# argriffing/raoteh

Hardware: AMD Instinct MI355X
Metric: site log-likelihoods/sec (batched tree pruning) (higher is better)
Workload: dtype f64; 1 GPU; c3: 61-state MG94 codon, 64-leaf balanced tree, 10000 sites/GPU, dense f64 leaf likelihood vectors; encoding=dense, sites_per_gpu=10000, sites_total=10000, states=61, leaves=64, edges=126, batches_rotated=3, reduce=none

## Files before the change

### include/raoteh_hip.h

```cpp
#ifndef RAOTEH_HIP_H
#define RAOTEH_HIP_H

#include <stdint.h>

#ifdef __cplusplus
extern "C" {
#endif

#define RT_OK                0
#define RT_ERR_INVALID      -1
#define RT_ERR_HIP          -2
#define RT_ERR_UNSUPPORTED  -3
#define RT_ERR_NOMEM        -4
#define RT_ERR_RCCL         -5
#define RT_ERR_SINGULAR     -6
#define RT_ERR_ZERO_PROB    -7

#define RT_MAX_STATES      128
#define RT_MAX_EXPECT_STATES 64
#define RT_MAX_EXPECT_STEP_STATES 128
#define RT_MAX_EXPM_STATES 128

#define RT_SITE_OK           0
#define RT_SITE_ZERO_PROB    1
// ... 53 lines not shown

int rt_mcy_esd_get_node_to_pmap(rt_ctx *ctx, int64_t nnodes, int64_t n,
            int64_t nsites, const int64_t *tree_csr_indices,
            const int64_t *tree_csr_indptr, const double *esd_transitions,
            const int64_t *state_mask, const double *obs_likelihood,
            double *subtree_probability);
int rt_mcy_esd_passes(rt_ctx *ctx, int64_t nnodes, int64_t n, int64_t nsites,
            const int64_t *tree_csr_indices, const int64_t *tree_csr_indptr,
            const double *esd_transitions, int64_t *state_mask,
            const double *obs_likelihood, double *subtree_probability);

int rt_mc0_esd_get_node_to_distn(rt_ctx *ctx, int64_t nnodes, int64_t n,
            int64_t nsites, const int64_t *tree_csr_indices,
            const int64_t *tree_csr_indptr, const double *esd_transitions,
            const double *root_distn, const double *subtree_probability,
            double *node_to_distn_array, int32_t *status);

int rt_mc0_esd_get_joint_endpoint_distn(rt_ctx *ctx, int64_t nnodes, int64_t n,
            int64_t nsites, const int64_t *tree_csr_indices,
            const int64_t *tree_csr_indptr, const double *esd_transitions,
            const double *subtree_probability, const double *node_to_distn_array,
            double *joint_distns);

int rt_mjp_esd_expectation_weights(rt_ctx *ctx, int64_t nnodes, int64_t n,
            int64_t nsites, const int64_t *tree_csr_indices,
            const int64_t *tree_csr_indptr, const double *esd_transitions,
            const double *root_distn, const int64_t *state_mask,
            const double *site_weights, double *edge_weights, int32_t *status);

int rt_mjp_esd_expectation_weights_obs(rt_ctx *ctx, int64_t nnodes, int64_t n,
            int64_t nsites, const int64_t *tree_csr_indices,
            const int64_t *tree_csr_indptr, const double *esd_transitions,
            const double *root_distn, int64_t nobs, const int64_t *obs_nodes, int kind,
            const void *data, const double *site_weights, double *edge_weights,
            int32_t *status);

int rt_mjp_frechet_statistics(rt_ctx *ctx, int64_t n, int64_t nedges, const double *Q,
            int64_t nq, const int64_t *q_index, const double *t, const double *W,
            double *dwell, double *trans);


int rt_model_create(rt_ctx *ctx, int64_t nnodes, int64_t n,
            const int64_t *tree_csr_indices, const int64_t *tree_csr_indptr,
            rt_model **model);
int rt_model_destroy(rt_model *model);

int rt_model_set_rates(rt_model *model, const double *Q, int64_t nq,
            const int64_t *node_q, const double *t);
int rt_model_set_rates_spectral(rt_model *model, const double *A, const double *lam,
            const double *B, const double *D, const double *t);
int rt_model_recompute_transitions(rt_model *model);
int rt_model_set_transitions(rt_model *model, const double *esd_transitions);
int rt_model_get_transitions(rt_model *model, double *esd_transitions);
int rt_model_get_expm_info(rt_model *model, int32_t *info );
int rt_model_set_root_distn(rt_model *model, const double *root_distn);

int rt_model_schedule_depth(const rt_model *model);
int rt_model_get_schedule(const rt_model *model, int32_t *ops, int64_t capacity,
            int64_t *nops);
int rt_build_schedule(int64_t nnodes, const int64_t *tree_csr_indices,
            const int64_t *tree_csr_indptr, int32_t *ops ,
            int32_t *depth);
int rt_set_option(const char *key, int64_t value);
int rt_ctx_set_option(rt_ctx *ctx, const char *key, int64_t value);
int rt_jit_source(int64_t nnodes, const int64_t *tree_csr_indices,
            const int64_t *tree_csr_indptr, int64_t n, int64_t nobs,
            const int64_t *obs_nodes, int64_t prefetch, char *buf, int64_t capacity);

int rt_sites_create(rt_model *model, int64_t nsites, int kind, int64_t nobs,
            const int64_t *obs_nodes, const void *data, rt_sites **sites);
int rt_sites_clone(rt_sites *sites, rt_sites **clone);
int rt_sites_jit_wait(rt_sites *sites);
int rt_jit_wait_all(void);
int rt_sites_destroy(rt_sites *sites);
int64_t rt_sites_device_bytes(const rt_sites *sites);
double rt_sites_jit_compile_seconds(const rt_sites *sites);
int rt_debug_jit_global(rt_sites *sites, const char *name, void *dst, int64_t bytes);
const char *rt_sites_kernel_name(const rt_sites *sites);

int rt_prune(rt_model *model, rt_sites *sites);
int rt_step(rt_model *model, rt_sites *sites, int recompute_transitions);
int rt_carry_combine_deal(int64_t nt, int64_t nblocks16, int64_t G, int root_halves,
            int rescale, int partitioned, int multi, int64_t *tile_of);
int rt_expect_step(rt_model *model, rt_sites *sites, int recompute_transitions,
            double *dwell, double *root_posterior, double *trans, int32_t *status);
#define RT_MAX_POSTERIOR_SETS 8
int rt_sites_posteriors(rt_model *model, rt_sites *sites, int recompute_transitions,
            int64_t n_node_sets, const uint64_t *node_sets,
            int64_t n_edge_sets, const uint64_t *edge_sets,
            int64_t n_marginal_nodes, const int64_t *marginal_nodes,
            double *node_values, double *edge_values, double *marginals, int32_t *status);
#define RT_MAX_BRANCH_COEFS 8
int rt_sites_branch_expectations(rt_model *model, rt_sites *sites, int recompute_transitions,
            int64_t n_coefs, const double *coefs, double *values, double *edge_sums,
            int32_t *status);
#define RT_MAX_PROFILE_POINTS 64
int rt_sites_branch_profiles(rt_model *model, rt_sites *sites, int recompute_transitions,
            int64_t npoints, const double *lengths, double *values, double *sums,
            int32_t *status);
int rt_model_get_branch_lengths(rt_model *model, double *t);
int rt_model_nni_moves(const rt_model *model, int32_t *moves, int64_t capacity, int64_t *nmoves);
int rt_tree_nni_moves(int64_t nnodes, const int64_t *tree_csr_indices, const int64_t *tree_csr_indptr,
            int32_t *moves, int64_t capacity, int64_t *nmoves);
int rt_sites_nni_scores(rt_model *model, rt_sites *sites, int recompute_transitions,
            int64_t npoints, const double *lengths, double *values, double *sums,
            int32_t *status);
#define RT_MAX_PLACE_FRACTIONS 8
#define RT_MAX_PLACE_PENDANT   16
int rt_sites_placements(rt_model *model, rt_sites *sites, int recompute_transitions,
            int64_t nqueries, int query_kind, const void *queries,
            int64_t nfractions, const double *fractions,
            int64_t npendant, const double *pendant,
            double *values, double *sums, int32_t *status);
int rt_model_spr_moves(const rt_model *model, int64_t radius, int32_t *moves, int64_t capacity,
            int64_t *nmoves);
int rt_tree_spr_moves(int64_t nnodes, const int64_t *tree_csr_indices, const int64_t *tree_csr_indptr,
            int64_t radius, int32_t *moves, int64_t capacity, int64_t *nmoves);
int rt_sites_spr_scores(rt_model *model, rt_sites *sites, int recompute_transitions,
            int64_t radius, int64_t nfractions, const double *fractions,
            double *values, double *sums, int32_t *status);
#define RT_MAX_SAMPLE_NODES 8192
int rt_sites_sample_states(rt_model *model, rt_sites *sites, int recompute_transitions,
            uint64_t seed, uint64_t first_draw, int64_t ndraws,
            uint8_t *states ,
            int32_t *status );
int rt_sample_states_draw_block(int64_t nnodes);
int rt_sites_map_states(rt_model *model, rt_sites *sites, int recompute_transitions,
            uint8_t *states      ,
            double  *log_joint   ,
            int32_t *status      );
#define RT_MAX_MAPPING_EVENTS 512
int rt_sites_sample_mappings(rt_model *model, rt_sites *sites, int recompute_transitions,
            uint64_t seed, uint64_t first_draw, int64_t ndraws,
            int64_t n_coefs, const double *coefs ,
            uint8_t *states  ,
            double *values   ,
            int32_t *counts  ,
            double *means    ,
            int32_t *status  );
int rt_sites_set_weights(rt_sites *sites, const double *weights);
int rt_sites_get_logliks(rt_sites *sites, double *loglik, int32_t *status);
int rt_sites_get_totals(rt_sites *sites, double totals[3]);

#define RT_MAX_RATE_SETS 64
int rt_model_set_rate_sets(rt_model *model, int64_t K, const double *Q, int64_t nq,
            const int64_t *node_q, const double *t);
int rt_step_multi(rt_model *model, rt_sites *sites, int recompute_transitions);
int rt_sites_get_multi_logliks(rt_sites *sites, double *loglik, int32_t *status);
int rt_sites_get_multi_totals(rt_sites *sites, double *totals, double *weighted_sums);
int rt_sites_multi_mixture(rt_sites *sites, const double *class_weights, double *loglik,
            int32_t *status, double totals[3]);
const char *rt_sites_multi_kernel_name(const rt_sites *sites);

int rt_partition_plan(const int32_t *site_set, int64_t nsites, int64_t nsets, int64_t granule,
            int64_t capacity, int64_t *order, int64_t *slot_of_site, uint8_t *is_pad,
            int32_t *granule_set, int64_t *run_begin, int64_t *padded);
int rt_sites_create_partitioned(rt_model *model, int64_t nsites, int kind, int64_t nobs,
            const int64_t *obs_nodes, const void *data, const int32_t *site_set, int64_t nsets,
            rt_sites **sites);
int rt_step_partitioned(rt_model *model, rt_sites *sites, int recompute_transitions);
int rt_sites_get_partition_totals(rt_sites *sites, double *totals, double *weighted_sums);
int rt_sites_branch_expectations_partitioned(rt_model *model, rt_sites *sites,
            int recompute_transitions, int64_t n_coefs, int coefs_per_set, const double *coefs,
            double *values, double *edge_sums, double *set_edge_sums, int32_t *status);
int rt_sites_branch_profiles_partitioned(rt_model *model, rt_sites *sites, int recompute_transitions,
            int64_t npoints, const double *factors, double *values, double *sums,
// ... 87 lines not shown
```

### raoteh_amd/_lib.py

```python
from __future__ import annotations

import ctypes
import os
from ctypes import (POINTER, c_char_p, c_double, c_int, c_int32,
                    c_int64, c_ubyte, c_void_p)

__all__ = ['HipLibraryError', 'RaotehHipError', 'lib', 'check', 'LIB_PATH']

LIB_PATH = os.environ.get(
    'RAOTEH_HIP_LIB',
    os.path.join(os.path.dirname(os.path.abspath(__file__)), 'libraoteh_hip.so'))

RT_OK = 0
RT_ERR_INVALID = -1
RT_ERR_HIP = -2
RT_ERR_UNSUPPORTED = -3
RT_ERR_NOMEM = -4
RT_ERR_RCCL = -5
RT_ERR_SINGULAR = -6
RT_ERR_ZERO_PROB = -7

RT_OBS_DENSE, RT_OBS_STATE, RT_OBS_MASK = 0, 1, 2
RT_K_EXPM, RT_K_PRUNE, RT_K_REDUCE, RT_K_COMBINE = 0, 1, 2, 3
RT_SITE_ZERO_PROB = 1
# ... 8 lines not shown
RT_MAX_EXPECT_STATES = 64
RT_MAX_EXPECT_STEP_STATES = 128
RT_MAX_RATE_SETS = 64


class HipLibraryError(ImportError):
    """libraoteh_hip.so is missing / not loadable (run __graft_entry__.build())."""


class RaotehHipError(RuntimeError):

    def __init__(self, code, message):
        RuntimeError.__init__(self, '%s (code %d)' % (message, code))
        self.code = code


_p_i64 = POINTER(c_int64)
_p_f64 = POINTER(c_double)
_p_i32 = POINTER(c_int32)

SIGNATURES = {
    'rt_version': (c_int, []),
    'rt_last_error': (c_char_p, []),
    'rt_device_count': (c_int, [POINTER(c_int)]),
    'rt_ctx_create': (c_int, [c_int, POINTER(c_void_p)]),
    'rt_ctx_destroy': (c_int, [c_void_p]),
    'rt_ctx_sync': (c_int, [c_void_p]),
    'rt_ctx_set_timing': (c_int, [c_void_p, c_int]),
    'rt_ctx_reset_timing': (c_int, [c_void_p]),
    'rt_ctx_kernel_time': (c_int, [c_void_p, c_int, POINTER(c_double),
                                   POINTER(c_int64), POINTER(c_char_p)]),
    'rt_expm': (c_int, [c_void_p, c_int64, c_int64, _p_f64, c_int64, _p_i64,
                        _p_f64, _p_f64, _p_i32]),
    'rt_lb_transition_matrix': (c_int, [c_void_p, c_int64, c_int64, _p_f64, _p_f64, _p_f64]),
    'rt_tmjp_get_inhomogeneous_mjp': (c_int, [c_int64, _p_i64, _p_i64, _p_i64, c_int64, _p_i64,
                                              _p_f64, c_double, c_double, c_int64, _p_i64,
                                              _p_f64]),
    'rt_mcy_get_node_to_pset': (c_int, [c_void_p, c_int64, c_int64, _p_i64, _p_i64, _p_i64,
                                        _p_i64, _p_i64]),
    'rt_get_node_to_set': (c_int, [c_void_p, c_int64, c_int64, _p_i64, _p_i64, _p_i64, _p_i64,
                                   _p_i64, _p_i64]),
    'rt_mcy_esd_get_node_to_pset': (c_int, [c_void_p, c_int64, c_int64, c_int64,
                                            _p_i64, _p_i64, _p_f64, _p_i64]),
    'rt_esd_get_node_to_set': (c_int, [c_void_p, c_int64, c_int64, c_int64,
                                       _p_i64, _p_i64, _p_f64, _p_i64]),
    'rt_mcy_esd_get_node_to_pmap': (c_int, [c_void_p, c_int64, c_int64, c_int64,
                                            _p_i64, _p_i64, _p_f64, _p_i64,
                                            _p_f64, _p_f64]),
    'rt_mcy_esd_passes': (c_int, [c_void_p, c_int64, c_int64, c_int64,
                                  _p_i64, _p_i64, _p_f64, _p_i64,
                                  _p_f64, _p_f64]),
    'rt_mc0_esd_get_node_to_distn': (c_int, [c_void_p, c_int64, c_int64, c_int64,
                                             _p_i64, _p_i64, _p_f64, _p_f64,
                                             _p_f64, _p_f64, _p_i32]),
    'rt_mc0_esd_get_joint_endpoint_distn': (c_int, [c_void_p, c_int64, c_int64,
                                                    c_int64, _p_i64, _p_i64,
                                                    _p_f64, _p_f64, _p_f64,
                                                    _p_f64]),
    'rt_mjp_esd_expectation_weights': (c_int, [c_void_p, c_int64, c_int64, c_int64,
                                               _p_i64, _p_i64, _p_f64, _p_f64, _p_i64,
                                               _p_f64, _p_f64, _p_i32]),
    'rt_mjp_esd_expectation_weights_obs': (c_int, [c_void_p, c_int64, c_int64, c_int64,
                                                   _p_i64, _p_i64, _p_f64, _p_f64, c_int64,
                                                   _p_i64, c_int, c_void_p, _p_f64, _p_f64,
                                                   _p_i32]),
    'rt_mjp_frechet_statistics': (c_int, [c_void_p, c_int64, c_int64, _p_f64, c_int64, _p_i64,
                                          _p_f64, _p_f64, _p_f64, _p_f64]),
    'rt_model_create': (c_int, [c_void_p, c_int64, c_int64, _p_i64, _p_i64,
                                POINTER(c_void_p)]),
    'rt_model_destroy': (c_int, [c_void_p]),
    'rt_model_set_rates': (c_int, [c_void_p, _p_f64, c_int64, _p_i64, _p_f64]),
    'rt_model_set_rates_spectral': (c_int, [c_void_p, _p_f64, _p_f64, _p_f64, _p_f64, _p_f64]),
    'rt_expm_spectral': (c_int, [c_void_p, c_int64, c_int64, _p_f64, _p_f64, _p_f64, _p_f64,
                                 _p_f64, _p_f64]),
    'rt_model_recompute_transitions': (c_int, [c_void_p]),
    'rt_model_set_transitions': (c_int, [c_void_p, _p_f64]),
    'rt_model_get_transitions': (c_int, [c_void_p, _p_f64]),
    'rt_model_get_expm_info': (c_int, [c_void_p, _p_i32]),
    'rt_model_set_root_distn': (c_int, [c_void_p, _p_f64]),
    'rt_model_schedule_depth': (c_int, [c_void_p]),
    'rt_model_get_schedule': (c_int, [c_void_p, _p_i32, c_int64, _p_i64]),
    'rt_build_schedule': (c_int, [c_int64, _p_i64, _p_i64, _p_i32, _p_i32]),
    'rt_carry_combine_deal': (c_int, [c_int64, c_int64, c_int64, c_int, c_int, c_int, c_int, _p_i64]),
    'rt_set_option': (c_int, [c_char_p, c_int64]),
    'rt_ctx_set_option': (c_int, [c_void_p, c_char_p, c_int64]),
    'rt_sites_jit_compile_seconds': (c_double, [c_void_p]),
    'rt_sites_kernel_name': (c_char_p, [c_void_p]),
    'rt_debug_jit_global': (c_int, [c_void_p, c_char_p, c_void_p, c_int64]),
    'rt_jit_source': (c_int, [c_int64, _p_i64, _p_i64, c_int64, c_int64, _p_i64, c_int64,
                              c_char_p, c_int64]),
    'rt_sites_create': (c_int, [c_void_p, c_int64, c_int, c_int64, _p_i64,
                                c_void_p, POINTER(c_void_p)]),
    'rt_sites_clone': (c_int, [c_void_p, POINTER(c_void_p)]),
    'rt_sites_jit_wait': (c_int, [c_void_p]),
    'rt_jit_wait_all': (c_int, []),
    'rt_expect_step': (c_int, [c_void_p, c_void_p, c_int, _p_f64, _p_f64, _p_f64, _p_i32]),
    'rt_sites_posteriors': (c_int, [c_void_p, c_void_p, c_int, c_int64, c_void_p, c_int64,
                                    c_void_p, c_int64, _p_i64, _p_f64, _p_f64, _p_f64, _p_i32]),
    'rt_sites_branch_expectations': (c_int, [c_void_p, c_void_p, c_int, c_int64, _p_f64, _p_f64,
                                             _p_f64, _p_i32]),
    'rt_sites_branch_profiles': (c_int, [c_void_p, c_void_p, c_int, c_int64, _p_f64, _p_f64,
                                         _p_f64, _p_i32]),
    'rt_model_get_branch_lengths': (c_int, [c_void_p, _p_f64]),
    'rt_model_nni_moves': (c_int, [c_void_p, _p_i32, c_int64, _p_i64]),
    'rt_tree_nni_moves': (c_int, [c_int64, _p_i64, _p_i64, _p_i32, c_int64, _p_i64]),
    'rt_sites_nni_scores': (c_int, [c_void_p, c_void_p, c_int, c_int64, _p_f64, _p_f64, _p_f64,
                                    _p_i32]),
    'rt_sites_placements': (c_int, [c_void_p, c_void_p, c_int, c_int64, c_int, c_void_p, c_int64,
                                    _p_f64, c_int64, _p_f64, _p_f64, _p_f64, _p_i32]),
    'rt_model_spr_moves': (c_int, [c_void_p, c_int64, _p_i32, c_int64, _p_i64]),
    'rt_tree_spr_moves': (c_int, [c_int64, _p_i64, _p_i64, c_int64, _p_i32, c_int64, _p_i64]),
    'rt_sites_spr_scores': (c_int, [c_void_p, c_void_p, c_int, c_int64, c_int64, _p_f64, _p_f64,
                                    _p_f64, _p_i32]),
    'rt_sites_sample_states': (c_int, [c_void_p, c_void_p, c_int, ctypes.c_uint64,
                                       ctypes.c_uint64, c_int64, POINTER(c_ubyte), _p_i32]),
    'rt_sample_states_draw_block': (c_int, [c_int64]),
    'rt_sites_map_states': (c_int, [c_void_p, c_void_p, c_int, POINTER(c_ubyte), _p_f64, _p_i32]),
    'rt_sites_sample_mappings': (c_int, [c_void_p, c_void_p, c_int, ctypes.c_uint64,
                                         ctypes.c_uint64, c_int64, c_int64, _p_f64,
                                         POINTER(c_ubyte), _p_f64, _p_i32, _p_f64, _p_i32]),
    'rt_sites_set_weights': (c_int, [c_void_p, _p_f64]),
    'rt_sites_destroy': (c_int, [c_void_p]),
    'rt_sites_device_bytes': (c_int64, [c_void_p]),
    'rt_prune': (c_int, [c_void_p, c_void_p]),
    'rt_step': (c_int, [c_void_p, c_void_p, c_int]),
    'rt_sites_get_logliks': (c_int, [c_void_p, _p_f64, _p_i32]),
    'rt_sites_get_totals': (c_int, [c_void_p, _p_f64]),
    'rt_model_set_rate_sets': (c_int, [c_void_p, c_int64, _p_f64, c_int64, _p_i64, _p_f64]),
    'rt_step_multi': (c_int, [c_void_p, c_void_p, c_int]),
    'rt_sites_get_multi_logliks': (c_int, [c_void_p, _p_f64, _p_i32]),
    'rt_sites_get_multi_totals': (c_int, [c_void_p, _p_f64, _p_f64]),
    'rt_sites_multi_mixture': (c_int, [c_void_p, _p_f64, _p_f64, _p_i32, _p_f64]),
    'rt_sites_multi_kernel_name': (c_char_p, [c_void_p]),
    'rt_partition_plan': (c_int, [_p_i32, c_int64, c_int64, c_int64, c_int64, _p_i64, _p_i64,
                                  POINTER(c_ubyte), _p_i32, _p_i64, _p_i64]),
    'rt_sites_create_partitioned': (c_int, [c_void_p, c_int64, c_int, c_int64, _p_i64, c_void_p,
                                            _p_i32, c_int64, POINTER(c_void_p)]),
    'rt_step_partitioned': (c_int, [c_void_p, c_void_p, c_int]),
    'rt_sites_get_partition_totals': (c_int, [c_void_p, _p_f64, _p_f64]),
    'rt_sites_partition_info': (c_int, [c_void_p, _p_i64, _p_i64, _p_i64]),
    'rt_sites_branch_expectations_partitioned': (c_int, [c_void_p, c_void_p, c_int, c_int64, c_int,
                                                         _p_f64, _p_f64, _p_f64, _p_f64, _p_i32]),
    'rt_sites_branch_profiles_partitioned': (c_int, [c_void_p, c_void_p, c_int, c_int64, _p_f64, _p_f64,
                                                     _p_f64, _p_f64, _p_i32]),
    'rt_sites_nni_scores_partitioned': (c_int, [c_void_p, c_void_p, c_int, c_int64, _p_f64, _p_f64,
                                                _p_f64, _p_f64, _p_i32]),
    'rt_sites_spr_scores_partitioned': (c_int, [c_void_p, c_void_p, c_int, c_int64, c_int64, _p_f64,
                                                _p_f64, _p_f64, _p_f64, _p_i32]),
    'rt_sites_placements_partitioned': (c_int, [c_void_p, c_void_p, c_int, c_int64, c_int, c_void_p,
                                                c_int64, _p_f64, c_int64, _p_f64, _p_f64, _p_f64,
                                                _p_f64, _p_f64, _p_i32]),
    'rt_sites_branch_expectations_mixture': (c_int, [c_void_p, c_void_p, c_int, _p_f64, c_int64, c_int,
                                                     _p_f64, _p_f64, _p_f64, _p_f64, _p_f64, _p_f64,
                                                     _p_f64, _p_i32]),
    'rt_sites_branch_profiles_mixture': (c_int, [c_void_p, c_void_p, c_int, _p_f64, c_int64, _p_f64,
                                                 _p_f64, _p_f64, _p_f64, _p_i32]),
    'rt_sites_nni_scores_mixture': (c_int, [c_void_p, c_void_p, c_int, _p_f64, c_int64, _p_f64,
                                            _p_f64, _p_f64, _p_f64, _p_i32]),
    'rt_sites_spr_scores_mixture': (c_int, [c_void_p, c_void_p, c_int, _p_f64, c_int64, c_int64,
                                            _p_f64, _p_f64, _p_f64, _p_f64, _p_i32]),
    'rt_sites_placements_mixture': (c_int, [c_void_p, c_void_p, c_int, _p_f64, c_int64, c_int,
                                            c_void_p, c_int64, _p_f64, c_int64, _p_f64, _p_f64,
                                            _p_f64, _p_f64, _p_f64, _p_i32]),
    'rt_comm_available': (c_int, []),
    'rt_comm_unique_id': (c_int, [POINTER(c_ubyte)]),
    'rt_comm_init': (c_int, [c_void_p, c_int, c_int, POINTER(c_ubyte)]),
# ... 69 lines not shown
```

### raoteh_amd/csrc/api.hip

```cpp
#include "common.h"
#include "partition_plan.h"

#include <algorithm>
#include <atomic>
#include <functional>
#include <cmath>
#include <cstdlib>


static thread_local char g_err[512] = "";

void rt_set_error(const char *fmt, ...)
{
    va_list ap;
    va_start(ap, fmt);
    vsnprintf(g_err, sizeof(g_err), fmt, ap);
    va_end(ap);
}

extern "C" const char *rt_last_error(void) { return g_err; }
extern "C" int rt_version(void) { return 100; }

extern "C" int rt_device_count(int *count)
{
// ... 271 lines not shown
        for (int64_t e = m->indptr[v]; e < m->indptr[v + 1]; ++e) {
            kids[(size_t)v].push_back((int32_t)m->indices[e]);
            m->parent[(size_t)m->indices[e]] = (int32_t)v;
        }
    std::vector<int> need((size_t)N, 0);
    for (int64_t v = N - 1; v >= 0; --v) {
        auto &k = kids[(size_t)v];
        if (k.empty()) continue;
        std::stable_sort(k.begin(), k.end(),
                         [&](int32_t a, int32_t b) { return need[a] > need[b]; });
        int nd = std::max(1, need[k[0]]);
        for (size_t i = 1; i < k.size(); ++i) nd = std::max(nd, 1 + need[k[i]]);
        need[(size_t)v] = nd;
    }
    m->ops.clear();
    m->ops.reserve((size_t)N);
    std::vector<int32_t> acc_slot((size_t)N, -1);
    std::vector<std::pair<int32_t, size_t>> stack;
    stack.emplace_back(0, 0);
    int sp = 0, maxsp = 0;
    while (!stack.empty()) {
        const int32_t v = stack.back().first;
        const size_t ci = stack.back().second;
        auto &k = kids[(size_t)v];
        if (ci < k.size()) {
            stack.back().second = ci + 1;
            stack.emplace_back(k[ci], 0);
            continue;
        }
        stack.pop_back();
        rt_op op;
        op.node = v;
        op.obs = -1;
        op.pop = k.empty() ? -1 : acc_slot[(size_t)v];
        if (!k.empty()) sp -= 1;
        if (stack.empty()) {
            op.dst = -1;
        } else {
            const int32_t p = stack.back().first;
            if (acc_slot[(size_t)p] < 0) {
                acc_slot[(size_t)p] = sp;
                op.dst = sp | 256;
                sp += 1;
                maxsp = std::max(maxsp, sp);
            } else {
                op.dst = acc_slot[(size_t)p];
            }
        }
        m->ops.push_back(op);
    }
    m->max_depth = maxsp;
}

extern "C" int rt_build_schedule(int64_t nnodes, const int64_t *idx, const int64_t *ptr,
                                 int32_t *ops, int32_t *depth)
{
    RT_REQUIRE(nnodes >= 1 && ptr && (idx || nnodes == 1) && ops, "bad arguments");
    RT_REQUIRE(ptr[0] == 0 && ptr[nnodes] == nnodes - 1,
               "tree_csr_indptr does not describe a tree");
    for (int64_t v = 0; v < nnodes; ++v)
        for (int64_t e = ptr[v]; e < ptr[v + 1]; ++e)
            RT_REQUIRE(idx[e] > v && idx[e] < nnodes, "children not in preorder");
    rt_model m;
    m.nnodes = nnodes;
    if (nnodes > 1) m.indices.assign(idx, idx + (nnodes - 1));
    m.indptr.assign(ptr, ptr + nnodes + 1);
    build_schedule(&m);
    memcpy(ops, m.ops.data(), m.ops.size() * sizeof(rt_op));
    if (depth) *depth = m.max_depth;
    return RT_OK;
}

static int64_t pfrag_doubles(const rt_model *m)
{
    const int64_t nops = (int64_t)m->ops.size();
    if (m->n <= 4) return (nops + 1) * m->n * m->n;
    const int64_t nt = (m->n + 15) / 16, kp = ((m->n + 3) / 4 + 1) / 2;
    return nops * nt * kp * 128;
}

static void rate_sets_release(rt_model *m)
{
    rt_rate_sets &r = m->multi;
    hipFree(r.d_Q); hipFree(r.d_qidx); hipFree(r.d_t); hipFree(r.d_info); hipFree(r.d_step_of_node);
    hipFree(r.d_P); hipFree(r.d_Pfrag); hipFree(r.d_Pquad); hipFree(r.d_Pcol);
    r = rt_rate_sets();
}

extern "C" int rt_model_destroy(rt_model *m)
{
    if (!m) return RT_OK;
    if (m->live_batches > 0) {
        rt_set_error("rt_model_destroy: %d site batch(es) of this model are still alive; "
                     "destroy them first", m->live_batches);
        return RT_ERR_INVALID;
    }
    m->ctx->live_models -= 1;
    hipSetDevice(m->ctx->device);
    rt_expect_state_release(m);
    rt_expect_lane_release(m);
    hipStreamSynchronize(m->ctx->stream);
    hipFree(m->d_indices); hipFree(m->d_indptr); hipFree(m->d_ops); hipFree(m->d_P);
    hipFree(m->d_Pfrag); hipFree(m->d_Pquad); hipFree(m->d_Pcol); hipFree(m->d_root); hipFree(m->d_Q); hipFree(m->d_spec); hipFree(m->d_qidx);
    hipFree(m->d_t); hipFree(m->d_info); hipFree(m->d_step_of_node);
    hipFree(m->d_qidx_step); hipFree(m->d_t_step);
    rate_sets_release(m);
    delete m;
    return RT_OK;
}

extern "C" int rt_model_create(rt_ctx *ctx, int64_t nnodes, int64_t n,
                               const int64_t *idx, const int64_t *ptr, rt_model **out)
{
    RT_REQUIRE(ctx && out, "null pointer");
    *out = nullptr;
    RT_REQUIRE(nnodes >= 1 && n >= 1, "bad sizes");
    RT_REQUIRE(n <= RT_MAX_STATES, "n=%lld > %d", (long long)n, RT_MAX_STATES);
    RT_REQUIRE(nnodes < (1ll << 30), "tree too large");
    RT_REQUIRE(ptr && (idx || nnodes == 1), "null array");
    RT_REQUIRE(ptr[0] == 0 && ptr[nnodes] == nnodes - 1,
               "tree_csr_indptr does not describe a tree");
    std::vector<char> seen((size_t)nnodes, 0);
    for (int64_t v = 0; v < nnodes; ++v) {
        RT_REQUIRE(ptr[v + 1] >= ptr[v], "tree_csr_indptr not monotone");
        for (int64_t e = ptr[v]; e < ptr[v + 1]; ++e) {
            RT_REQUIRE(idx[e] > v && idx[e] < nnodes,
                       "child index %lld of node %lld is not in preorder",
                       (long long)idx[e], (long long)v);
            RT_REQUIRE(!seen[(size_t)idx[e]], "node %lld has two parents",
                       (long long)idx[e]);
            seen[(size_t)idx[e]] = 1;
        }
    }
    RT_HIP(hipSetDevice(ctx->device));
    rt_model *m = new (std::nothrow) rt_model();
    if (!m) return RT_ERR_NOMEM;
    m->ctx = ctx;
    ctx->live_models += 1;
    m->nnodes = nnodes;
    m->n = n;
    if (nnodes > 1) m->indices.assign(idx, idx + (nnodes - 1));
    m->indptr.assign(ptr, ptr + nnodes + 1);
    build_schedule(m);
    const size_t nn = (size_t)n * n;
    hipError_t e = hipMalloc((void **)&m->d_indices, std::max<size_t>(8, (nnodes - 1) * 8));
    if (e == hipSuccess) e = hipMalloc((void **)&m->d_indptr, (nnodes + 1) * 8);
    if (e == hipSuccess) e = hipMalloc((void **)&m->d_ops, m->ops.size() * sizeof(rt_op));
    if (e == hipSuccess) e = hipMalloc((void **)&m->d_P, nnodes * nn * 8);
    if (e == hipSuccess) e = hipMalloc((void **)&m->d_Pfrag, pfrag_doubles(m) * 8);
    if (e == hipSuccess) e = hipMemset(m->d_Pfrag, 0, pfrag_doubles(m) * 8);
    if (e == hipSuccess && n > 4 && n <= 32) {
        const size_t bytes = m->ops.size() * (size_t)rt_quad_stride((int)n) * 8;
        e = hipMalloc((void **)&m->d_Pquad, bytes);
        if (e == hipSuccess) e = hipMemset(m->d_Pquad, 0, bytes);
    }
    if (e == hipSuccess) e = hipMalloc((void **)&m->d_root, n * 8);
    if (e == hipSuccess) e = hipMalloc((void **)&m->d_qidx, nnodes * 4);
    if (e == hipSuccess) e = hipMalloc((void **)&m->d_t, nnodes * 8);
    if (e == hipSuccess) e = hipMalloc((void **)&m->d_info, nnodes * 8);
    if (e == hipSuccess && n <= 4) e = hipMalloc((void **)&m->d_qidx_step, nnodes * 4);
    if (e == hipSuccess && n <= 4) e = hipMalloc((void **)&m->d_t_step, nnodes * 8);
    if (e == hipSuccess && nnodes > 1)
        e = hipMemcpy(m->d_indices, idx, (nnodes - 1) * 8, hipMemcpyHostToDevice);
    if (e == hipSuccess) e = hipMemcpy(m->d_indptr, ptr, (nnodes + 1) * 8, hipMemcpyHostToDevice);
    if (e == hipSuccess)
        e = hipMemcpy(m->d_ops, m->ops.data(), m->ops.size() * sizeof(rt_op),
                      hipMemcpyHostToDevice);
    std::vector<int32_t> step_of((size_t)nnodes, -1);
    for (size_t k = 0; k < m->ops.size(); ++k) step_of[(size_t)m->ops[k].node] = (int32_t)k;
    if (e == hipSuccess) e = hipMalloc((void **)&m->d_step_of_node, nnodes * 4);
    if (e == hipSuccess)
        e = hipMemcpy(m->d_step_of_node, step_of.data(), nnodes * 4, hipMemcpyHostToDevice);
    if (e == hipSuccess) e = hipMemset(m->d_P, 0, nnodes * nn * 8);
    if (e == hipSuccess) e = hipMemset(m->d_info, 0, nnodes * 8);
    std::vector<double> ones((size_t)n, 1.0);
    if (e == hipSuccess) e = hipMemcpy(m->d_root, ones.data(), n * 8, hipMemcpyHostToDevice);
    if (e != hipSuccess) {
        rt_set_error("rt_model_create: %s", hipGetErrorString(e));
        rt_model_destroy(m);
        return e == hipErrorOutOfMemory ? RT_ERR_NOMEM : RT_ERR_HIP;
    }
    *out = m;
    return RT_OK;
}

static int model_upload_edge_parameters(rt_model *m, const std::vector<int32_t> &qi,
                                        const std::vector<double> &tt)
{
    if (qi != m->h_qidx) {
        RT_HIP(hipMemcpy(m->d_qidx, qi.data(), m->nnodes * 4, hipMemcpyHostToDevice));
        m->h_qidx = qi;
        if (m->d_qidx_step) {
            std::vector<int32_t> by_step(m->ops.size());
            for (size_t k = 0; k < m->ops.size(); ++k) by_step[k] = qi[(size_t)m->ops[k].node];
            RT_HIP(hipMemcpy(m->d_qidx_step, by_step.data(), by_step.size() * 4, hipMemcpyHostToDevice));
        }
    }
    if (tt != m->h_t) {
        RT_HIP(hipMemcpy(m->d_t, tt.data(), m->nnodes * 8, hipMemcpyHostToDevice));
        m->h_t = tt;
        if (m->d_t_step) {
            std::vector<double> by_step(m->ops.size());
            for (size_t k = 0; k < m->ops.size(); ++k) by_step[k] = tt[(size_t)m->ops[k].node];
            RT_HIP(hipMemcpy(m->d_t_step, by_step.data(), by_step.size() * 8, hipMemcpyHostToDevice));
        }
    }
    return RT_OK;
}

static int model_run_expm(rt_model *m)
{
    rt_reduce_args red;
    const bool carry = rt_take_pending_reduce(m->ctx, &red);
    if (m->spectral) {
        RT_TRY(rt_flush_combine(m->ctx));
        const size_t nn = (size_t)m->n * m->n;
        RT_TRY(rt_launch_spectral(m->ctx, m->n, m->nnodes, m->d_spec, m->d_spec + 2 * nn,
                                  m->d_spec + nn, m->spectral_has_D ? m->d_spec + 2 * nn + m->n
                                                                    : nullptr,
                                  m->d_qidx, m->d_t, m->d_P, m->d_info, m->d_step_of_node,
                                  m->n <= 4 ? 0 : 1, m->d_Pfrag, carry ? &red : nullptr,
                                  m->d_Pquad));
        m->have_P = true;
        m->rates_current = true;
        m->frag_dirty = false;
        return rt_model_pack_pcol(m);
    }
    rt_combine_args comb;
    rt_sites *carried = nullptr;
    RT_TRY(rt_take_pending_combine(m->ctx, rt_expm_carry_groups(m->ctx, m->n, m->nnodes, carry,
                                                                m->d_Pquad != nullptr),
                                   carry ? &red : nullptr, &comb, &carried));
    const int erc = rt_launch_expm(m->ctx, m->n, m->nnodes, m->d_Q, m->d_qidx, m->d_t, m->d_P,
                                   m->d_info, m->d_step_of_node, m->n <= 4 ? 0 : 1, m->d_Pfrag,
                                   carry ? &red : nullptr, m->d_Pquad, 0, carried ? &comb : nullptr);
    if (carried) RT_TRY(rt_carried_combine_done(m->ctx, carried, erc == RT_OK));
    RT_TRY(erc);
    m->have_P = true;
    m->rates_current = true;
    m->frag_dirty = false;
    return rt_model_pack_pcol(m);
}

extern "C" int rt_model_set_rates(rt_model *m, const double *Q, int64_t nq,
                                  const int64_t *node_q, const double *t)
{
    RT_REQUIRE(m && Q && t, "null pointer");
    RT_REQUIRE(nq >= 1, "nq must be >= 1");
    if (m->n > RT_MAX_EXPM_STATES) {
        rt_set_error("expm: n=%lld > %d", (long long)m->n, RT_MAX_EXPM_STATES);
        return RT_ERR_UNSUPPORTED;
    }
    RT_HIP(hipSetDevice(m->ctx->device));
    const size_t nn = (size_t)m->n * m->n;
    std::vector<int32_t> qi((size_t)m->nnodes);
    std::vector<double> tt((size_t)m->nnodes);
    qi[0] = -1;
    tt[0] = 0.0;
    for (int64_t v = 1; v < m->nnodes; ++v) {
        const int64_t q = node_q ? node_q[v] : 0;
        RT_REQUIRE(q >= 0 && q < nq, "node_q[%lld]=%lld out of range", (long long)v,
                   (long long)q);
        RT_REQUIRE(std::isfinite(t[v]), "branch length of node %lld is not finite",
                   (long long)v);
        qi[(size_t)v] = (int32_t)q;
        tt[(size_t)v] = t[v];
    }
    if (nq > m->q_capacity) {
        hipFree(m->d_Q);
        m->d_Q = nullptr;
        m->q_capacity = 0;
        RT_HIP(hipMalloc((void **)&m->d_Q, nq * nn * 8));
        m->q_capacity = nq;
    }
    hipStream_t st = m->ctx->stream;
    RT_HIP(hipStreamSynchronize(st));
    RT_HIP(hipMemcpy(m->d_Q, Q, nq * nn * 8, hipMemcpyHostToDevice));
    RT_TRY(model_upload_edge_parameters(m, qi, tt));
    m->spectral = false;
    return model_run_expm(m);
}

extern "C" int rt_model_set_rates_spectral(rt_model *m, const double *A, const double *lam,
                                           const double *B, const double *D, const double *t)
{
    RT_REQUIRE(m && A && lam && B && t, "null pointer");
    if (m->n > 64) {
        rt_set_error("spectral reconstruction: n=%lld > 64", (long long)m->n);
        return RT_ERR_UNSUPPORTED;
    }
    RT_HIP(hipSetDevice(m->ctx->device));
    const size_t n = (size_t)m->n, nn = n * n;
    std::vector<int32_t> qi((size_t)m->nnodes, 0);
    std::vector<double> tt((size_t)m->nnodes);
    qi[0] = -1;
    tt[0] = 0.0;
    for (int64_t v = 1; v < m->nnodes; ++v) {
        RT_REQUIRE(std::isfinite(t[v]), "branch length of node %lld is not finite", (long long)v);
        tt[(size_t)v] = t[v];
    }
    for (size_t i = 0; i < n; ++i)
        RT_REQUIRE(std::isfinite(lam[i]) && (!D || D[i] >= 0.0), "eigenvalue / weight %zu", i);
    if (!m->d_spec) RT_HIP(hipMalloc((void **)&m->d_spec, (2 * nn + 2 * n) * 8));
    RT_HIP(hipStreamSynchronize(m->ctx->stream));
    RT_HIP(hipMemcpy(m->d_spec, A, nn * 8, hipMemcpyHostToDevice));
    RT_HIP(hipMemcpy(m->d_spec + nn, B, nn * 8, hipMemcpyHostToDevice));
    RT_HIP(hipMemcpy(m->d_spec + 2 * nn, lam, n * 8, hipMemcpyHostToDevice));
    if (D) RT_HIP(hipMemcpy(m->d_spec + 2 * nn + n, D, n * 8, hipMemcpyHostToDevice));
    m->spectral_has_D = D != nullptr;
    RT_TRY(model_upload_edge_parameters(m, qi, tt));
    m->spectral = true;
    return model_run_expm(m);
}

extern "C" int rt_expm_spectral(rt_ctx *ctx, int64_t n, int64_t count, const double *A,
                                const double *lam, const double *B, const double *D,
                                const double *t, double *P)
{
    RT_REQUIRE(ctx, "null context");
    RT_REQUIRE(n >= 1 && count >= 0, "bad sizes");
    RT_REQUIRE(A && lam && B && t && P, "null array");
    if (n > 64) {
        rt_set_error("spectral reconstruction: n=%lld > 64", (long long)n);
        return RT_ERR_UNSUPPORTED;
    }
    if (count == 0) return RT_OK;
    RT_HIP(hipSetDevice(ctx->device));
    const size_t nn = (size_t)n * n;
    auto up = [](size_t b) { return (b + 255) & ~(size_t)255; };
    const size_t o_A = 0, o_B = o_A + up(nn * 8), o_lam = o_B + up(nn * 8), o_D = o_lam + up(n * 8),
                 o_t = o_D + up(n * 8), o_P = o_t + up(count * 8), total = o_P + up(count * nn * 8);
    RT_TRY(rt_scratch_reserve(ctx, total));
    unsigned char *base = ctx->d_scratch;
    double *dA = (double *)(base + o_A), *dB = (double *)(base + o_B), *dl = (double *)(base + o_lam),
           *dD = (double *)(base + o_D), *dt = (double *)(base + o_t), *dP = (double *)(base + o_P);
    int rc = RT_OK;
    hipError_t e = hipMemcpyAsync(dA, A, nn * 8, hipMemcpyHostToDevice, ctx->stream);
    if (e == hipSuccess) e = hipMemcpyAsync(dB, B, nn * 8, hipMemcpyHostToDevice, ctx->stream);
    if (e == hipSuccess) e = hipMemcpyAsync(dl, lam, n * 8, hipMemcpyHostToDevice, ctx->stream);
    if (e == hipSuccess && D) e = hipMemcpyAsync(dD, D, n * 8, hipMemcpyHostToDevice, ctx->stream);
    if (e == hipSuccess) e = hipMemcpyAsync(dt, t, count * 8, hipMemcpyHostToDevice, ctx->stream);
    if (e == hipSuccess)
        rc = rt_launch_spectral(ctx, n, count, dA, dl, dB, D ? dD : nullptr, nullptr, dt, dP, nullptr,
                                nullptr, 0, nullptr);
    if (e == hipSuccess && rc == RT_OK)
        e = hipMemcpyAsync(P, dP, count * nn * 8, hipMemcpyDeviceToHost, ctx->stream);
    if (e == hipSuccess && rc == RT_OK) e = hipStreamSynchronize(ctx->stream);
    if (rc != RT_OK) return rc;
    if (e != hipSuccess) {
        rt_set_error("rt_expm_spectral: %s", hipGetErrorString(e));
        return RT_ERR_HIP;
    }
    return RT_OK;
}


static int64_t rate_sets_steps(const rt_model *m)
{
    return (int64_t)m->ops.size() + (m->n <= 4 ? 1 : 0);
}

static int rate_sets_reserve(rt_model *m, int64_t K, int64_t nq)
{
    rt_rate_sets &r = m->multi;
    const int64_t n = m->n, N = m->nnodes, nn = n * n, nops = (int64_t)m->ops.size();
    if (K * nq > r.q_capacity) {
        RT_HIP(hipStreamSynchronize(m->ctx->stream));
        hipFree(r.d_Q);
        r.d_Q = nullptr;
        r.q_capacity = 0;
        RT_HIP(hipMalloc((void **)&r.d_Q, (size_t)(K * nq * nn) * 8));
        r.q_capacity = K * nq;
    }
    if (K <= r.capacity) return RT_OK;
    RT_HIP(hipStreamSynchronize(m->ctx->stream));
    double *keep_Q = r.d_Q;
    const int64_t keep_cap = r.q_capacity;
    r.d_Q = nullptr;
    const uint64_t epoch = r.epoch;
    rate_sets_release(m);
    r.d_Q = keep_Q;
    r.q_capacity = keep_cap;
    r.epoch = epoch + 1;
    r.P_stride = N * nn;
    r.frag_stride = pfrag_doubles(m);
    r.quad_stride = m->d_Pquad ? nops * (int64_t)rt_quad_stride((int)n) : 0;
    r.pcol_stride = nops * n * 16 * ((n + 15) / 16);
    hipError_t e = hipMalloc((void **)&r.d_qidx, (size_t)(K * N) * 4);
    if (e == hipSuccess) e = hipMalloc((void **)&r.d_t, (size_t)(K * N) * 8);
    if (e == hipSuccess) e = hipMalloc((void **)&r.d_info, (size_t)(K * N) * 8);
    if (e == hipSuccess) e = hipMalloc((void **)&r.d_step_of_node, (size_t)(K * N) * 4);
    if (e == hipSuccess) e = hipMalloc((void **)&r.d_P, (size_t)(K * r.P_stride) * 8);
    if (e == hipSuccess) e = hipMalloc((void **)&r.d_Pfrag, (size_t)(K * r.frag_stride) * 8);
    if (e == hipSuccess) e = hipMemset(r.d_Pfrag, 0, (size_t)(K * r.frag_stride) * 8);
    if (e == hipSuccess && r.quad_stride) {
        e = hipMalloc((void **)&r.d_Pquad, (size_t)(K * r.quad_stride) * 8);
        if (e == hipSuccess) e = hipMemset(r.d_Pquad, 0, (size_t)(K * r.quad_stride) * 8);
    }
    if (e == hipSuccess) e = hipMemset(r.d_info, 0, (size_t)(K * N) * 8);
    std::vector<int32_t> son((size_t)(K * N));
    const int64_t steps = rate_sets_steps(m);
    for (int64_t k = 0; k < K; ++k)
        for (size_t j = 0; j < m->ops.size(); ++j)
            son[(size_t)(k * N + m->ops[j].node)] = (int32_t)(k * steps + (int64_t)j);
    if (e == hipSuccess)
        e = hipMemcpy(r.d_step_of_node, son.data(), son.size() * 4, hipMemcpyHostToDevice);
    if (e == hipSuccess) e = hipDeviceSynchronize();
    if (e != hipSuccess) {
        rt_set_error("rt_model_set_rate_sets: %s", hipGetErrorString(e));
        rate_sets_release(m);
        m->multi.epoch = epoch + 1;
        return e == hipErrorOutOfMemory ? RT_ERR_NOMEM : RT_ERR_HIP;
    }
    r.capacity = K;
    return RT_OK;
}

static int rate_sets_pack_pcol(rt_model *m, bool fresh)
{
    rt_rate_sets &r = m->multi;
    if (!m->d_Pcol || m->n <= 4 || r.K <= 0) return RT_OK;
    if (r.pcol_capacity < r.capacity) {
        RT_HIP(hipStreamSynchronize(m->ctx->stream));
        hipFree(r.d_Pcol);
        r.d_Pcol = nullptr;
        r.pcol_capacity = 0;
        RT_HIP(hipMalloc((void **)&r.d_Pcol, (size_t)(r.capacity * r.pcol_stride) * 8));
        r.pcol_capacity = r.capacity;
        fresh = true;
    }
    if (!fresh) return RT_OK;
    return rt_pack_pcol_sets(m, r.K, r.d_P, r.P_stride, r.d_Pcol, r.pcol_stride);
}

static int rate_sets_run_expm(rt_model *m)
{
    rt_rate_sets &r = m->multi;
    RT_TRY(rt_launch_expm(m->ctx, m->n, r.K * m->nnodes, r.d_Q, r.d_qidx, r.d_t, r.d_P, r.d_info,
                          r.d_step_of_node, m->n <= 4 ? 0 : 1, r.d_Pfrag, nullptr, r.d_Pquad,
                          m->nnodes));
    return rate_sets_pack_pcol(m, true);
}

int rt_rate_sets_recompute(rt_model *m)
{
    RT_REQUIRE(m->multi.K > 0, "rt_model_set_rate_sets has not been called");
    return rate_sets_run_expm(m);
}

extern "C" int rt_model_set_rate_sets(rt_model *m, int64_t K, const double *Q, int64_t nq,
                                      const int64_t *node_q, const double *t)
{
    RT_REQUIRE(m && Q && t, "null pointer");
    RT_REQUIRE(K >= 1 && K <= RT_MAX_RATE_SETS, "K=%lld rate sets: 1..%d", (long long)K,
               RT_MAX_RATE_SETS);
    RT_REQUIRE(nq >= 1, "nq must be >= 1");
    if (m->n > RT_MAX_EXPM_STATES) {
        rt_set_error("expm: n=%lld > %d", (long long)m->n, RT_MAX_EXPM_STATES);
        return RT_ERR_UNSUPPORTED;
    }
    RT_HIP(hipSetDevice(m->ctx->device));
    const int64_t N = m->nnodes;
    const size_t nn = (size_t)m->n * m->n;
    std::vector<int32_t> qi((size_t)(K * N));
    std::vector<double> tt((size_t)(K * N));
    for (int64_t k = 0; k < K; ++k) {
        qi[(size_t)(k * N)] = -1;
        tt[(size_t)(k * N)] = 0.0;
        for (int64_t v = 1; v < N; ++v) {
            const int64_t q = node_q ? node_q[v] : 0;
            RT_REQUIRE(q >= 0 && q < nq, "node_q[%lld]=%lld out of range", (long long)v, (long long)q);
            RT_REQUIRE(std::isfinite(t[k * N + v]),
                       "branch length of node %lld in rate set %lld is not finite", (long long)v,
                       (long long)k);
            qi[(size_t)(k * N + v)] = (int32_t)(k * nq + q);
            tt[(size_t)(k * N + v)] = t[k * N + v];
        }
    }
    RT_TRY(rate_sets_reserve(m, K, nq));
    rt_rate_sets &r = m->multi;
    RT_HIP(hipStreamSynchronize(m->ctx->stream));
    RT_HIP(hipMemcpy(r.d_Q, Q, (size_t)(K * nq) * nn * 8, hipMemcpyHostToDevice));
    RT_HIP(hipMemcpy(r.d_qidx, qi.data(), qi.size() * 4, hipMemcpyHostToDevice));
    RT_HIP(hipMemcpy(r.d_t, tt.data(), tt.size() * 8, hipMemcpyHostToDevice));
    if (K != r.K) r.epoch += 1;
    r.K = K;
    r.nq = nq;
    r.h_node_q.assign((size_t)N, -1);
    for (int64_t v = 1; v < N; ++v) r.h_node_q[(size_t)v] = node_q ? (int32_t)node_q[v] : 0;
    return rate_sets_run_expm(m);
}

extern "C" int rt_model_recompute_transitions(rt_model *m)
{
    RT_REQUIRE(m, "null model");
    RT_REQUIRE(m->d_Q || m->spectral, "rt_model_set_rates has not been called");
    RT_HIP(hipSetDevice(m->ctx->device));
    return model_run_expm(m);
}

extern "C" int rt_model_set_transitions(rt_model *m, const double *esd)
{
    RT_REQUIRE(m && esd, "null pointer");
    RT_HIP(hipSetDevice(m->ctx->device));
    RT_HIP(hipStreamSynchronize(m->ctx->stream));
    RT_HIP(hipMemcpy(m->d_P, esd, (size_t)m->nnodes * m->n * m->n * 8,
                     hipMemcpyHostToDevice));
    m->have_P = true;
    m->rates_current = false;
    m->frag_dirty = true;
    return rt_launch_pfrag(m);
}

extern "C" int rt_model_get_transitions(rt_model *m, double *esd)
{
    RT_REQUIRE(m && esd, "null pointer");
    RT_REQUIRE(m->have_P, "the model has no transition matrices yet");
    RT_HIP(hipSetDevice(m->ctx->device));
    RT_HIP(hipStreamSynchronize(m->ctx->stream));
    RT_HIP(hipMemcpy(esd, m->d_P, (size_t)m->nnodes * m->n * m->n * 8,
                     hipMemcpyDeviceToHost));
    return RT_OK;
}

extern "C" int rt_model_get_expm_info(rt_model *m, int32_t *info)
{
    RT_REQUIRE(m && info, "null pointer");
    RT_HIP(hipSetDevice(m->ctx->device));
    RT_HIP(hipStreamSynchronize(m->ctx->stream));
    RT_HIP(hipMemcpy(info, m->d_info, (size_t)m->nnodes * 8, hipMemcpyDeviceToHost));
    for (int64_t v = 1; v < m->nnodes; ++v)
        if (info[2 * v] < 0) {
            rt_set_error("expm: the matrix of the edge above node %lld has a non-finite entry or "
                         "norm (Taylor scheme), or its Pade denominator is singular "
                         "(RAOTEH_EXPM=pade)", (long long)v);
            return RT_ERR_SINGULAR;
        }
    return RT_OK;
}

extern "C" int rt_model_set_root_distn(rt_model *m, const double *root_distn)
{
    RT_REQUIRE(m, "null model");
    RT_HIP(hipSetDevice(m->ctx->device));
    std::vector<double> w((size_t)m->n, 1.0);
    if (root_distn) w.assign(root_distn, root_distn + m->n);
    RT_TRY(rt_flush_pending(m->ctx));
    RT_HIP(hipStreamSynchronize(m->ctx->stream));
    RT_HIP(hipMemcpy(m->d_root, w.data(), m->n * 8, hipMemcpyHostToDevice));
    return RT_OK;
}

extern "C" int rt_model_schedule_depth(const rt_model *m)
{
    return m ? m->max_depth : -1;
}


static std::atomic<int> g_force_generic{0};
static std::atomic<int> g_jit{-1};
static const int64_t RT_JIT_MIN_WORK = 65536;
static std::atomic<int> g_jit_block_sites{0};
static std::atomic<int> g_jit_async{1};
static std::atomic<int> g_rescale{0};
static std::atomic<int> g_leaf_state_kernels{1};
// ... 1936 lines not shown
```

### raoteh_amd/csrc/common.h

```cpp
#pragma once

#include <hip/hip_runtime.h>
#include <hip/hip_ext.h>

#include <cstdarg>
#include <cstdint>
#include <cstdio>
#include <cstring>
#include <memory>
#include <string>
#include <type_traits>
#include <vector>

#include "../../include/raoteh_hip.h"


void rt_set_error(const char *fmt, ...);

#define RT_HIP(call)                                                          \
    do {                                                                      \
        hipError_t e_ = (call);                                               \
        if (e_ != hipSuccess) {                                               \
            rt_set_error("%s failed: %s (%s:%d)", #call,                      \
                         hipGetErrorString(e_), __FILE__, __LINE__);          \
// ... 30 lines not shown
    {
        for (void *&q : ptrs) if (q == p) q = nullptr;
        return p;
    }
};

struct post_plan {
    size_t total = 0;
    size_t take(size_t bytes)
    {
        const size_t o = total;
        total += (bytes + 255) / 256 * 256;
        return o;
    }
};
template <int LO, int HI, class F>
inline int post_dispatch(int v, F &&f)
{
    if constexpr (LO > HI) return RT_ERR_UNSUPPORTED;
    else return v == LO ? f(std::integral_constant<int, LO>()) : post_dispatch<LO + 1, HI>(v, f);
}

struct rt_jit_job;


struct rt_timing_slot {
    std::vector<std::pair<hipEvent_t, hipEvent_t>> pending;
    std::vector<hipEvent_t> pool;
    double total_ms = 0.0;
    int64_t launches = 0;
    int64_t seen = 0;
    char name[64] = "";
};

static const int RT_TOTALS_SLOTS = 4096;

struct rt_ctx {
    int device = 0;
    hipStream_t stream = nullptr;
    int num_cus = 0;
    bool timing = false;
    int timing_period = 1;
    rt_timing_slot slots[RT_K_COUNT];
    hipEvent_t ev_start = nullptr, ev_stop = nullptr;
    double *d_totals_arena = nullptr;
    std::vector<int> totals_free;
    hipEvent_t ev_reduced = nullptr;
    hipEvent_t comm_events[8] = {};
    int comm_event_next = 0;
    unsigned char *d_scratch = nullptr;
    size_t scratch_bytes = 0;
    void *comm = nullptr;
    hipStream_t comm_stream = nullptr;
    void *rccl = nullptr;
    int opt_force_generic = -2;
    int opt_jit = -2;
    int opt_jit_block_sites = -2;
    int opt_jit_async = -2;
    int opt_rescale = -2;
    int opt_leaf_state_kernels = -2;
    struct rt_sites *pending_reduce = nullptr;
    struct rt_sites *pending_combine = nullptr;
    size_t expm_attr_lds = 0;
    size_t expm_ts_attr_lds[8] = {0, 0, 0, 0, 0, 0, 0, 0};
    size_t expm_split_attr_lds = 0;
    size_t expm_w8_attr_lds[3] = {0, 0, 0};
    size_t expm_wide_attr_lds[8] = {0, 0, 0, 0, 0, 0, 0, 0};
    double *d_expm_scratch = nullptr;
    void *expect_cache = nullptr;
    size_t expm_scratch_bytes = 0;
    int live_models = 0, live_chains = 0;
};
static const int RT_OPT_UNSET = -2;

static const int RT_FAST_MAX_DEPTH = 16;

struct rt_op {
    int32_t node;
    int32_t obs;
    int32_t pop;
    int32_t dst;
};

struct rt_rate_sets {
    int64_t K = 0;
    int64_t capacity = 0;
    int64_t nq = 0, q_capacity = 0;
    uint64_t epoch = 0;
    double *d_Q = nullptr;
    int32_t *d_qidx = nullptr;
    double *d_t = nullptr;
    std::vector<int32_t> h_node_q;
    int32_t *d_info = nullptr;
    int32_t *d_step_of_node = nullptr;
    double *d_P = nullptr;
    double *d_Pfrag = nullptr, *d_Pquad = nullptr, *d_Pcol = nullptr;
    int64_t pcol_capacity = 0;
    int64_t P_stride = 0, frag_stride = 0, quad_stride = 0, pcol_stride = 0;
};

struct rt_model {
    rt_ctx *ctx = nullptr;
    int64_t nnodes = 0;
    int64_t n = 0;
    std::vector<int64_t> indices, indptr;
    std::vector<int32_t> parent;
    std::vector<rt_op> ops;
    std::vector<int32_t> h_qidx;
    std::vector<double> h_t;
    int max_depth = 0;
    int64_t *d_indices = nullptr, *d_indptr = nullptr;
    rt_op *d_ops = nullptr;
    double *d_P = nullptr;
    double *d_Pfrag = nullptr;
    double *d_Pquad = nullptr;
    double *d_Pcol = nullptr;
    double *d_root = nullptr;
    double *d_spec = nullptr;
    bool spectral = false, spectral_has_D = false;
    double *d_Q = nullptr;
    int64_t q_capacity = 0;
    int32_t *d_qidx = nullptr;
    double *d_t = nullptr;
    int32_t *d_info = nullptr;
    int32_t *d_step_of_node = nullptr;
    int32_t *d_qidx_step = nullptr;
    double *d_t_step = nullptr;
    bool have_P = false;
    bool rates_current = false;
    bool frag_dirty = true;
    int live_batches = 0;
    void *expect_state = nullptr;
    void *expect_lane_state = nullptr;
    rt_rate_sets multi;
};

enum { RT_LAYOUT_LANE = 0, RT_LAYOUT_MFMA = 1 };

struct rt_partition {
    int64_t nsites = 0;
    int64_t nsets = 0, G = 0, padded = 0;
    int64_t *d_order = nullptr;
    int64_t *d_slot_of_site = nullptr;
    uint8_t *d_is_pad = nullptr;
    int32_t *d_granule_set = nullptr;
    int64_t *d_run_begin = nullptr;
    std::vector<int64_t> run_begin;
    double *d_loglik = nullptr;
    int32_t *d_status = nullptr;
    int nblocks = 1;
    double *d_totals = nullptr;
    bool stepped = false;
    uint64_t epoch = 0;
    int64_t model_K = 0;
    int64_t device_bytes = 0;
};

struct rt_sites {
    rt_model *model = nullptr;
    int64_t nsites = 0;
    int64_t nobs = 0;
    int layout = RT_LAYOUT_LANE;
    bool lane_dma = false;
    int lane_ring = 8;
    bool mfma_solo = false;
    int64_t nblocks = 0;
    int64_t obs_bytes = 0;
    std::vector<int32_t> node_obs;
    std::vector<rt_op> ops;
    rt_op *d_ops = nullptr;
    int32_t *d_lane_ops = nullptr;
    int lane_stack_slots = 1;
    int64_t lane_nprog = 0;
    double *d_obs = nullptr;
    double *d_loglik = nullptr;
    int32_t *d_status = nullptr;
    double *d_partial = nullptr;
    int64_t npartials = 0;
    double *d_totals = nullptr;
    int totals_slot = -1;
    hipEvent_t ev_comm_done = nullptr;
    bool comm_pending = false;
    void *jit_fn = nullptr;
    int jit_prefetch = 0;
    int jit_lookahead = 1;
    int block_sites = 64;
    int jit_waves = 1;
    int jit_tiles = 1;
    bool jit_quad = false;
    bool jit_fused = false;
    double *d_partial_alt = nullptr;
    bool jit_halves = false;
    void *jit_combine = nullptr;
    double *d_half = nullptr;
    bool jit_fold = false;
    bool jit_teams = false;
    int *d_half_count = nullptr;
    bool interp_halves = false;
    bool rescale = false;
    int32_t *d_lane_ops_a = nullptr, *d_lane_ops_b = nullptr;
    int32_t *d_down_meta = nullptr;
    int down_slots = 0;
    int half_nops[2] = {0, 0};
    int half_rec1 = 0, half_kobs1 = 0, half_kroot = -1;
// ... 9 lines not shown
    int jit_kind = 0;
    bool keep_raw = false;
    void *d_raw = nullptr;
    int *d_raw_src = nullptr;
    struct { int S = 64, WG = 1, D = 1, LA = 1, compact = 0; bool fuse = false; } jit_lane;
    bool sparse_ok = false;
    bool sparse_pairs = false;
    bool jit_sparse = false;
    bool jit_pipe = false;
    unsigned *d_leafw = nullptr;
    double *d_weights = nullptr;
    unsigned char *d_sets = nullptr;
    rt_sites *expect_twin = nullptr;
    bool obs_borrowed = false;
    bool counted = false;
    bool pruned = false;
    char kernel_name[64] = "";
    int64_t multi_capacity = 0;
    int64_t multi_padded = 0, multi_npartials = 0;
    int64_t multi_K = 0;
    uint64_t multi_epoch = 0;
    void *multi_last_fn = nullptr;
    bool multi_last_valid = false;
    double *d_mloglik = nullptr;
    int32_t *d_mstatus = nullptr;
    double *d_mpartial = nullptr;
    double *d_mtotals = nullptr;
    char multi_kernel_name[80] = "";
    int multi_state = 0;
    void *multi_fn = nullptr, *multi_combine = nullptr, *multi_for = nullptr;
    std::shared_ptr<rt_jit_job> multi_job;
    std::string multi_src;
    double *d_mhalf = nullptr;
    int *d_mhalf_count = nullptr;
    int64_t multi_half_stride = 0, multi_count_stride = 0, multi_half_capacity = 0;
    double jit_compile_s = 0.0;
    rt_partition *part = nullptr;
};


void rt_time_begin(rt_ctx *ctx, int kernel, const char *name, hipEvent_t *start);
void rt_time_end(rt_ctx *ctx, int kernel, hipEvent_t start);
bool rt_time_extra_begin(rt_ctx *ctx, int kernel, const char *name, hipEvent_t *a, hipEvent_t *b);
void rt_time_extra_end(rt_ctx *ctx, int kernel, hipEvent_t a, hipEvent_t b);

struct rt_reduce_args {
    const double *partial = nullptr;
    long npartials = 0;
    double *totals = nullptr;
    double nsites = 0.0;
};
struct rt_combine_args {
    const double *halfbuf = nullptr;
    const double *obs = nullptr;
    int K = 0, KP = 0, kroot = -1;
    const double *root_w = nullptr;
    int n = 0;
    double *loglik = nullptr;
    int *status = nullptr;
    double *partial = nullptr;
    long nsites = 0, nblocks16 = 0;
    int wave_slots = 1;
};
__host__ __device__ inline long rt_carry_tile(long wg, int k, long G, long nblocks16)
{
    const long t = wg + (long)k * G;
    return t < nblocks16 ? t : -1;
}
inline bool rt_carry_combine_plan(int64_t nt, int64_t nblocks16, int64_t G, bool halves, bool rescale,
                                  bool partitioned, bool multi, int64_t *tile_of = nullptr)
{
    const bool ok = nt == 4 && halves && !rescale && !partitioned && !multi && G >= 1 &&
                    nblocks16 >= 1 && nblocks16 <= 4 * G;
    if (ok && tile_of)
        for (int64_t wg = 0; wg < G; ++wg)
            for (int k = 0; k < 4; ++k) tile_of[4 * wg + k] = rt_carry_tile((long)wg, k, (long)G, (long)nblocks16);
    return ok;
}
int64_t rt_expm_carry_groups(rt_ctx *ctx, int64_t n, int64_t count, bool with_reduce, bool quad);
int rt_expm_wide_launch(rt_ctx *ctx, int nt, bool split2, size_t grid, int64_t n, const double *d_Q,
                        const int *d_qidx, const double *d_t, double *d_P, int *d_info,
                        const int *d_step_of_node, int frag_kind, double *d_Pfrag,
                        const rt_reduce_args &red);
int rt_launch_expm(rt_ctx *ctx, int64_t n, int64_t count, const double *d_Q,
                   const int32_t *d_qidx, const double *d_t, double *d_P,
                   int32_t *d_info, const int32_t *d_step_of_node, int frag_kind,
                   double *d_Pfrag, const rt_reduce_args *fused_reduce = nullptr,
                   double *d_Pquad = nullptr, int64_t variant_count = 0,
                   const rt_combine_args *carried_combine = nullptr);
int rt_launch_spectral(rt_ctx *ctx, int64_t n, int64_t count, const double *d_A,
                       const double *d_lam, const double *d_B, const double *d_D,
                       const int32_t *d_qidx, const double *d_t, double *d_P, int32_t *d_info,
                       const int32_t *d_step_of_node, int frag_kind, double *d_Pfrag,
                       const rt_reduce_args *fused_reduce = nullptr, double *d_Pquad = nullptr);
bool rt_take_pending_reduce(rt_ctx *ctx, rt_reduce_args *out);
int rt_flush_reduce(rt_ctx *ctx);
int rt_take_pending_combine(rt_ctx *ctx, int64_t G, const rt_reduce_args *red, rt_combine_args *out,
                            struct rt_sites **taken);
int rt_carried_combine_done(rt_ctx *ctx, struct rt_sites *s, bool launched);
int rt_flush_combine(rt_ctx *ctx);
int rt_flush_pending(rt_ctx *ctx);
int rt_flush_pending_of(rt_ctx *ctx, const struct rt_sites *s);
#define RT_LAUNCH_TIMED(ctx, kern, grid, block, lds, ...)                               \
    do {                                                                                \
        if ((ctx)->ev_start)                                                            \
            hipExtLaunchKernelGGL(kern, grid, block, lds, (ctx)->stream,                \
                                  (ctx)->ev_start, (ctx)->ev_stop, 0, __VA_ARGS__);     \
        else                                                                            \
            hipLaunchKernelGGL(kern, grid, block, lds, (ctx)->stream, __VA_ARGS__);     \
    } while (0)
int rt_launch_pfrag(rt_model *m);
int rt_model_pack_pcol(rt_model *m);
int rt_model_need_pcol(rt_model *m);
int rt_pack_pcol_sets(rt_model *m, int64_t sets, const double *d_P, int64_t P_stride, double *d_Pcol,
                      int64_t pcol_stride);
struct rt_prune_view {
    const double *P = nullptr, *Pfrag = nullptr, *Pquad = nullptr, *Pcol = nullptr;
    double *loglik = nullptr;
    int32_t *status = nullptr;
    double *partial = nullptr;
    const int32_t *granule_set = nullptr;
    int64_t frag_stride = 0, pcol_stride = 0;
    bool defer_combine = false;
};
int64_t rt_lane_reg_granule(const rt_model *m);
int rt_partition_stage1_blocks(int64_t longest_run);
int64_t rt_partition_totals_doubles(int64_t nsets, int nblocks);
int rt_partition_reduce_launch(rt_ctx *ctx, const rt_partition *part, const double *d_loglik,
                               const int32_t *d_status, const double *d_weights,
                               double *d_batch_totals);
int64_t rt_multi_totals_doubles(int64_t K, int64_t nsites);
int rt_multi_reduce_launch(rt_ctx *ctx, int64_t K, const double *d_partial, int64_t npartials,
                           const double *d_loglik, const int32_t *d_status, int64_t padded,
                           int64_t nsites, const double *d_weights, double *d_totals,
                           double *d_wsums);
int rt_multi_mixture_launch(rt_ctx *ctx, int64_t K, const double *d_logc, const double *d_loglik,
                            const int32_t *d_status, int64_t padded, int64_t nsites,
                            const double *d_weights, double *d_out, int32_t *d_out_status,
                            double *d_partial, double *d_totals);
int rt_launch_prune(rt_model *m, rt_sites *s, bool defer_reduce = false, bool fuse_expm = false,
                    const struct rt_prune_view *view = nullptr);
struct rt_fuse_args {
    rt_reduce_args red;
    bool expm = false;
};
std::string rt_jit_lane_source(const std::vector<rt_op> &ops, int n, int K, int D, int LA,
                               int S, int WG, int compact = 0, bool fuse = false);
std::string rt_jit_mfma_source(const std::vector<rt_op> &ops, int n, int K, int T, int D, int LA,
                               bool quad = false, int sparse = 0);
std::string rt_jit_mfma_split_source(const std::vector<rt_op> &ops, int n, int K, int T, int D,
                                     int LA, int sparse = 0);
bool rt_jit_fold_enabled();
std::string rt_jit_mfma_split_pipelined_source(const std::vector<rt_op> &ops, int n, int K, int T,
                                               int D, int LA, bool halves = false,
                                               int sparse = 0, bool multi = false,
                                               bool teams = false);
bool rt_jit_teams_possible(int n, int T, int sparse);
int rt_jit_teams_env();
void rt_jit_root_halves(const std::vector<rt_op> &ops, int *stepsA, int *stepsB);
bool rt_split_at_root(const std::vector<rt_op> &ops, std::vector<rt_op> *A, std::vector<rt_op> *B);
int rt_jit_companion(const rt_ctx *ctx, void *fn, const char *name, void **out);
int rt_jit_get(rt_ctx *ctx, const std::string &src, void **fn, bool mfma = false,
               double *compile_s = nullptr);
std::shared_ptr<rt_jit_job> rt_jit_start(rt_ctx *ctx, std::vector<std::string> sources, bool mfma);
bool rt_jit_job_done(rt_jit_job *job, bool wait);
void rt_jit_job_result(rt_jit_job *job, int *rc, int *chosen, double *seconds, std::string *error);
void rt_jit_join_all(const rt_ctx *ctx);
int rt_jit_jobs_pending();
int rt_jit_cached(const rt_ctx *ctx, const std::string &src);
int rt_sites_jit_poll(rt_sites *s, bool wait);
void rt_jit_ref(const rt_ctx *ctx, void *fn, int delta);
int rt_jit_verified(const rt_ctx *ctx, void *fn);
// ... 66 lines not shown
```

### raoteh_amd/csrc/expm.hip

```cpp
#include "common.h"

#include <algorithm>
#include "reduce.h"
#include "site_epilogue.h"
#include "combine_body.inc"

#include <cstdlib>

namespace {

__constant__ double c_theta[5] = {1.495585217958292e-2, 2.539398330063230e-1,
                                  9.504178996162932e-1, 2.097847961257068e0,
                                  5.371920351148152e0};
__constant__ double c_b3[4] = {120., 60., 12., 1.};
__constant__ double c_b5[6] = {30240., 15120., 3360., 420., 30., 1.};
__constant__ double c_b7[8] = {17297280., 8648640., 1995840., 277200.,
                               25200., 1512., 56., 1.};
__constant__ double c_b9[10] = {17643225600., 8821612800., 2075673600.,
                                302702400., 30270240., 2162160., 110880.,
                                3960., 90., 1.};
__constant__ double c_b13[14] = {64764752532480000., 32382376266240000.,
                                 7771770303897600., 1187353796428800.,
                                 129060195264000., 10559470521600.,
                                 670442572800., 33522128640., 1323241920.,
// ... 304 lines not shown
            switch ((k + 1) >> 4) {
            case 0:
#pragma unroll
                for (int a = 0; a < 4; ++a) nb[16 * a] = g[a][0];
                break;
            case 1:
#pragma unroll
                for (int a = 0; a < 4; ++a) nb[16 * a] = g[a][1];
                break;
            case 2:
#pragma unroll
                for (int a = 0; a < 4; ++a) nb[16 * a] = g[a][2];
                break;
            default:
#pragma unroll
                for (int a = 0; a < 4; ++a) nb[16 * a] = g[a][3];
                break;
            }
        }
        __syncthreads();
    }
    __syncthreads();
    if (ibuf[2]) {
        for (int e = tid; e < nn; e += TPB) Pb[e] = __builtin_nan("");
        if (info && tid == 0) info[2 * b] = -1;
        return;
    }
#pragma unroll
    for (int a = 0; a < 4; ++a) {
        const int i = ri + 16 * a;
        if (i < n) {
            const double d = dinv[i];
            const int xr = kof[i];
#pragma unroll
            for (int bb = 0; bb < 8; ++bb) {
                const int c = ci + 16 * bb;
                if (c >= n && c < 2 * n) Xb[xr * ld + (c - n)] = g[a][bb] * d;
            }
        }
    }
    __syncthreads();
    for (int q = 0; q < s; ++q) lds_matmul(Xb, Xb, Xb, n, ld, NT, KS);

    RT_FOR_EACH_ELEMENT(i, j, o_unused_) {
        const int e = i * n + j;
        Pb[e] = Xb[i * ld + j];
    }
    if (step >= 0 && frag_kind == 0) {
        RT_FOR_EACH_ELEMENT(i, j, o_unused_) {
            const int e = i * n + j;
            Pfrag[(long)step * nn + e] = Xb[i * ld + j];
        }
    } else if (step >= 0 && frag_kind == 1) {
        const int KP = (KS + 1) / 2;
        const int total = NT * KP * 128;
        for (int e = tid; e < total; e += TPB) {
            const int e2 = e & 1;
            const int ln = (e >> 1) & 63;
            const int q = (e >> 7) % KP;
            const int mm = (e >> 7) / KP;
            const int row = 16 * mm + (ln & 15);
            const int col = 4 * (2 * q + e2) + (ln >> 4);
            Pfrag[(long)step * total + e] = (row < n && col < n) ? Xb[row * ld + col] : 0.0;
        }
        if (Pquad) {
            const int tq = KS * KS * 16;
            for (int e = tid; e < tq; e += TPB) {
                const int i = e & 3, k = (e >> 2) & 3, blk = e >> 4;
                const int row = 4 * (blk / KS) + i, col = 4 * (blk % KS) + k;
                Pquad[(long)step * rt_quad_stride(n) + e] = (row < n && col < n) ? Xb[row * ld + col] : 0.0;
            }
        }
    }
}


__constant__ double c_theta_taylor[5] = {1.3863479e-5, 9.0656564e-3, 8.9577602e-2,
                                         2.9961589e-1, 6.4108352e-1};
__constant__ double c_inv_fact[16] = {
    1.0, 1.0, 0.5, 1.0 / 6.0, 1.0 / 24.0, 1.0 / 120.0, 1.0 / 720.0, 1.0 / 5040.0,
    1.0 / 40320.0, 1.0 / 362880.0, 1.0 / 3628800.0, 1.0 / 39916800.0, 1.0 / 479001600.0,
    1.0 / 6227020800.0, 1.0 / 87178291200.0, 1.0 / 1307674368000.0};

template <int NT>
struct lane_tiles {
    double v[(NT + 1) / 2][(NT + 1) / 2][4];
};

template <int NT>
__device__ __forceinline__ void load_tiles(const double *M, lane_tiles<NT> &t)
{
    constexpr int RH = (NT + 1) / 2;
    constexpr int LD = 16 * NT + 1;
    const int lane = threadIdx.x & 63;
    const int wave = __builtin_amdgcn_readfirstlane(threadIdx.x >> 6);
    const int wr = wave >> 1, wc = wave & 1;
    const int lr = lane & 15, lq = lane >> 4;
#pragma unroll
    for (int u = 0; u < RH; ++u)
#pragma unroll
        for (int v = 0; v < RH; ++v) {
            const int m = wr * RH + u, j = wc * RH + v;
            const bool ok = m < NT && j < NT;
#pragma unroll
            for (int r = 0; r < 4; ++r)
                t.v[u][v][r] = ok ? M[(16 * m + 4 * r + lq) * LD + 16 * j + lr] : 0.0;
        }
}

template <int NT>
__device__ __forceinline__ void mm_blocked(const double *X, const double *Y, double *C,
                                           const double *cf, const double *P1, const double *P2,
                                           const lane_tiles<NT> *R1 = nullptr,
                                           const lane_tiles<NT> *R2 = nullptr,
                                           lane_tiles<NT> *out = nullptr,
                                           const double *top = nullptr, double *C2 = nullptr)
{
    constexpr int RH = (NT + 1) / 2;
    constexpr int LD = 16 * NT + 1;
    constexpr int KS = 4 * NT;
    const int lane = threadIdx.x & 63;
    const int wave = __builtin_amdgcn_readfirstlane(threadIdx.x >> 6);
    const int wr = wave >> 1, wc = wave & 1;
    const int lr = lane & 15, lq = lane >> 4;
    double4_t acc[RH][RH];
    const double *ap[RH];
    const double *bp[RH];
    bool rok[RH], cok[RH];
#pragma unroll
    for (int u = 0; u < RH; ++u) {
        const int m = wr * RH + u, j = wc * RH + u;
        rok[u] = m < NT;
        cok[u] = j < NT;
        ap[u] = X + (16 * (rok[u] ? m : 0) + lr) * LD + lq;
        bp[u] = Y + lq * LD + 16 * (cok[u] ? j : 0) + lr;
#pragma unroll
        for (int v = 0; v < RH; ++v) acc[u][v] = (double4_t){0.0, 0.0, 0.0, 0.0};
    }
    if (cf) {
        const double c0 = cf[0], c1 = cf[1], c2 = cf[2];
#pragma unroll
        for (int u = 0; u < RH; ++u)
#pragma unroll
            for (int v = 0; v < RH; ++v)
                if (rok[u] && cok[v]) {
                    const int m = wr * RH + u, j = wc * RH + v;
                    const int col = 16 * j + lr;
#pragma unroll
                    for (int r = 0; r < 4; ++r) {
                        const int row = 16 * m + 4 * r + lq;
                        const int o = row * LD + col;
                        double w = c1 * (R1 ? R1->v[u][v][r] : P1[o]);
                        if (R2) w = fma(c2, R2->v[u][v][r], w);
                        else if (P2) w = fma(c2, P2[o], w);
                        if (row == col && (double)row < cf[3]) w += c0;
                        acc[u][v][r] = w;
                    }
                }
    }
    double a0[RH], b0[RH], a1[RH], b1[RH];
#pragma unroll
    for (int u = 0; u < RH; ++u) {
        a0[u] = ap[u][0];
        b0[u] = bp[u][0];
        a1[u] = ap[u][KS > 1 ? 4 : 0];
        b1[u] = bp[u][KS > 1 ? 4 * LD : 0];
    }
    for (int kk = 0; kk < KS; ++kk) {
        const int kn = kk + 2 < KS ? kk + 2 : KS - 1;
        double a2[RH], b2[RH];
#pragma unroll
        for (int u = 0; u < RH; ++u) { a2[u] = ap[u][4 * kn]; b2[u] = bp[u][4 * kn * LD]; }
        __builtin_amdgcn_sched_barrier(0);
#pragma unroll
        for (int u = 0; u < RH; ++u)
#pragma unroll
            for (int v = 0; v < RH; ++v)
                acc[u][v] = __builtin_amdgcn_mfma_f64_16x16x4f64(a0[u], b0[v], acc[u][v], 0, 0, 0);
        __builtin_amdgcn_sched_barrier(0);
#pragma unroll
        for (int u = 0; u < RH; ++u) { a0[u] = a1[u]; b0[u] = b1[u]; a1[u] = a2[u]; b1[u] = b2[u]; }
    }
    if (out) {
#pragma unroll
        for (int u = 0; u < RH; ++u)
#pragma unroll
            for (int v = 0; v < RH; ++v)
#pragma unroll
                for (int r = 0; r < 4; ++r) out->v[u][v][r] = acc[u][v][r];
    }
    __syncthreads();
#pragma unroll
    for (int u = 0; u < RH; ++u)
#pragma unroll
        for (int v = 0; v < RH; ++v)
            if (rok[u] && cok[v]) {
                const int m = wr * RH + u, j = wc * RH + v;
                const int col = 16 * j + lr;
#pragma unroll
                for (int r = 0; r < 4; ++r) {
                    const int row = 16 * m + 4 * r + lq;
                    C[row * LD + col] = acc[u][v][r];
                    if (top) {
                        double w = top[1] * R1->v[u][v][r];
                        w = fma(top[2], R2->v[u][v][r], w);
                        w = fma(top[3], acc[u][v][r], w);
                        C2[row * LD + col] = w + ((row == col && (double)row < top[4]) ? top[0] : 0.0);
                    }
                }
            }
    __syncthreads();
}

struct half_tiles {
    double v[2][4];
};

__device__ __forceinline__ void load_half_tiles(const double *M, half_tiles &t, int h)
{
    constexpr int LD = 65;
    const int lane = threadIdx.x & 63;
    const int wave = __builtin_amdgcn_readfirstlane(threadIdx.x >> 6);
    const int lr = lane & 15, lq = lane >> 4;
#pragma unroll
    for (int v = 0; v < 2; ++v)
#pragma unroll
        for (int r = 0; r < 4; ++r)
            t.v[v][r] = M[(16 * wave + 4 * r + lq) * LD + 16 * (2 * h + v) + lr];
}

__device__ unsigned long long rt_expm_fine[8];
#define RT_FINE(k) if (fine && threadIdx.x == 0) rt_expm_fine[k] = __builtin_readcyclecounter()

__device__ __forceinline__ void mm_half(const double *X, const double *Y, double *C,
                                        double c0, double c1, double c2, double nd,
                                        const half_tiles &R1, const half_tiles &R2, int h,
                                        bool fine = false)
{
    RT_FINE(0);
    constexpr int LD = 65, KS = 16;
    const int lane = threadIdx.x & 63;
    const int wave = __builtin_amdgcn_readfirstlane(threadIdx.x >> 6);
    const int lr = lane & 15, lq = lane >> 4;
    double4_t acc[2];
    const double *ap = X + (16 * wave + lr) * LD + lq;
    const double *bp = Y + lq * LD + 32 * h + lr;
    double a0 = ap[0], b00 = bp[0], b01 = bp[16];
    double a1 = ap[4], b10 = bp[4 * LD], b11 = bp[4 * LD + 16];
#pragma unroll
    for (int v = 0; v < 2; ++v) {
        const int col = 16 * (2 * h + v) + lr;
#pragma unroll
        for (int r = 0; r < 4; ++r) {
            const int row = 16 * wave + 4 * r + lq;
            double w = c1 * R1.v[v][r];
            w = fma(c2, R2.v[v][r], w);
            if (row == col && (double)row < nd) w += c0;
            acc[v][r] = w;
        }
    }
    RT_FINE(1);
#pragma unroll
    for (int kk = 0; kk < KS; ++kk) {
        const int kn = kk + 2 < KS ? kk + 2 : KS - 1;
        const double a2 = ap[4 * kn], b20 = bp[4 * kn * LD], b21 = bp[4 * kn * LD + 16];
        __builtin_amdgcn_sched_barrier(0);
        acc[0] = __builtin_amdgcn_mfma_f64_16x16x4f64(a0, b00, acc[0], 0, 0, 0);
        acc[1] = __builtin_amdgcn_mfma_f64_16x16x4f64(a0, b01, acc[1], 0, 0, 0);
        __builtin_amdgcn_sched_barrier(0);
        a0 = a1; b00 = b10; b01 = b11;
        a1 = a2; b10 = b20; b11 = b21;
    }
    RT_FINE(2);
    __syncthreads();
    RT_FINE(3);
#pragma unroll
    for (int v = 0; v < 2; ++v) {
        const int col = 16 * (2 * h + v) + lr;
#pragma unroll
        for (int r = 0; r < 4; ++r) C[(16 * wave + 4 * r + lq) * LD + col] = acc[v][r];
    }
    RT_FINE(4);
    __syncthreads();
    RT_FINE(5);
}

template <int NT>
__device__ __forceinline__ void wave8_tiles(int wave, int &m, int &j0, int &nc)
{
    if (NT == 4) { m = wave >> 1; j0 = 2 * (wave & 1); nc = 2; }
    else if (wave < 6) { m = wave / 3; j0 = wave - 3 * m; nc = 1; }
    else { m = 2; j0 = wave == 6 ? 0 : 2; nc = wave == 6 ? 2 : 1; }
}

template <int NT>
__device__ __forceinline__ void load_left8(const double *X, int m, double (&a)[4 * NT])
{
    constexpr int LD = 16 * NT + 1;
    const int lane = threadIdx.x & 63;
    const double *ap = X + (16 * m + (lane & 15)) * LD + (lane >> 4);
#pragma unroll
    for (int kk = 0; kk < 4 * NT; ++kk) a[kk] = ap[4 * kk];
}

template <int NT>
__device__ __forceinline__ void load_tiles8(const double *M, half_tiles &t, int m, int j0, int nc)
{
    constexpr int LD = 16 * NT + 1;
    const int lane = threadIdx.x & 63;
    const int lr = lane & 15, lq = lane >> 4;
#pragma unroll
    for (int v = 0; v < 2; ++v)
#pragma unroll
        for (int r = 0; r < 4; ++r)
            t.v[v][r] = v < nc ? M[(16 * m + 4 * r + lq) * LD + 16 * (j0 + v) + lr] : 0.0;
}

template <int NT, int NC>
__device__ __forceinline__ void mm8(const double (&a)[4 * NT], const double *Y, double *C,
                                    int m, int j0, int nc_wave, bool seed, double c0, double c1,
                                    double c2, double nd, const half_tiles *R1,
                                    const half_tiles *R2, half_tiles *out = nullptr,
                                    const double *top = nullptr, double *C2 = nullptr,
                                    bool fine = false)
{
    RT_FINE(0);
    constexpr int LD = 16 * NT + 1, KS = 4 * NT;
    const int nc = NC ? NC : nc_wave;
    const int lane = threadIdx.x & 63;
    const int lr = lane & 15, lq = lane >> 4;
    const double *bp = Y + lq * LD + 16 * j0 + lr;
    const int o1 = nc > 1 ? 16 : 0;
    double b00 = bp[0], b01 = bp[o1];
    double b10 = bp[4 * LD], b11 = bp[4 * LD + o1];
    double4_t acc[2];
#pragma unroll
    for (int v = 0; v < 2; ++v) {
        acc[v] = (double4_t){0.0, 0.0, 0.0, 0.0};
        if (seed && v < nc) {
            const int col = 16 * (j0 + v) + lr;
#pragma unroll
            for (int r = 0; r < 4; ++r) {
                const int row = 16 * m + 4 * r + lq;
                double w = c1 * R1->v[v][r];
                w = fma(c2, R2->v[v][r], w);
                if (row == col && (double)row < nd) w += c0;
                acc[v][r] = w;
            }
        }
    }
    RT_FINE(1);
#pragma unroll
    for (int kk = 0; kk < KS; ++kk) {
        const int kn = kk + 2 < KS ? kk + 2 : KS - 1;
        const double b20 = bp[4 * kn * LD], b21 = bp[4 * kn * LD + o1];
        __builtin_amdgcn_sched_barrier(0);
        acc[0] = __builtin_amdgcn_mfma_f64_16x16x4f64(a[kk], b00, acc[0], 0, 0, 0);
        if (NC != 1 && nc > 1)
            acc[1] = __builtin_amdgcn_mfma_f64_16x16x4f64(a[kk], b01, acc[1], 0, 0, 0);
        __builtin_amdgcn_sched_barrier(0);
        b00 = b10; b01 = b11;
        b10 = b20; b11 = b21;
    }
    RT_FINE(2);
    if (out) {
#pragma unroll
        for (int v = 0; v < 2; ++v)
#pragma unroll
            for (int r = 0; r < 4; ++r) out->v[v][r] = acc[v][r];
    }
    __syncthreads();
    RT_FINE(3);
#pragma unroll
    for (int v = 0; v < 2; ++v)
        if (v < nc) {
            const int col = 16 * (j0 + v) + lr;
#pragma unroll
            for (int r = 0; r < 4; ++r) {
                const int row = 16 * m + 4 * r + lq;
                C[row * LD + col] = acc[v][r];
                if (top) {
                    double w = top[1] * R1->v[v][r];
                    w = fma(top[2], R2->v[v][r], w);
                    w = fma(top[3], acc[v][r], w);
                    C2[row * LD + col] = w + ((row == col && (double)row < top[4]) ? top[0] : 0.0);
                }
            }
        }
    RT_FINE(4);
    __syncthreads();
    RT_FINE(5);
}

__device__ int rt_expm_trace_on = 0;
__device__ unsigned long long rt_expm_trace[8];
#define RT_EXPM_STAMP(k)                                                              \
    if (trace_on && blockIdx.x == (SPLIT ? 2 : 1) && threadIdx.x == 0)                \
        rt_expm_trace[k] = __builtin_readcyclecounter()

template <int NT, bool GLOBAL, bool SPLIT = false, int WAVES = 4>
__global__ void __launch_bounds__(64 * WAVES)
expm_taylor_kernel(int n, const double *__restrict__ Q, const int *__restrict__ qidx,
                   const double *__restrict__ tt, double *__restrict__ P,
                   int *__restrict__ info, const int *__restrict__ step_of_node,
                   int frag_kind, double *__restrict__ Pfrag, double *__restrict__ Pquad,
                   double *__restrict__ scratch, rt_reduce_args red)
#define RT_EXPM_CARRY 0
#include "expm_taylor_body.inc"
#undef RT_EXPM_CARRY

template <int NT, bool GLOBAL, bool SPLIT, int WAVES>
__global__ void __launch_bounds__(64 * WAVES)
expm_taylor_carry_kernel(int n, const double *__restrict__ Q, const int *__restrict__ qidx,
                         const double *__restrict__ tt, double *__restrict__ P,
                         int *__restrict__ info, const int *__restrict__ step_of_node,
                         int frag_kind, double *__restrict__ Pfrag, double *__restrict__ Pquad,
                         double *__restrict__ scratch, rt_reduce_args red, rt_combine_args comb)
#define RT_EXPM_CARRY 1
#include "expm_taylor_body.inc"
#undef RT_EXPM_CARRY


#define RT_SHARED_SOURCE(...) __VA_ARGS__
#include "expm_small.inc"
#undef RT_SHARED_SOURCE

template <int N>
__global__ void __launch_bounds__(256)
expm_small_kernel(int count, const double *__restrict__ Q, const int *__restrict__ qidx,
                  const double *__restrict__ tt, double *__restrict__ P,
                  int *__restrict__ info, const int *__restrict__ step_of_node,
                  double *__restrict__ Pfrag, rt_reduce_args red)
{
    if (red.partial && blockIdx.x == gridDim.x - 1) {
        rt_reduce_partials_body(red.partial, red.npartials, red.totals, red.nsites);
        return;
    }
    const int b = blockIdx.x * 256 + threadIdx.x;
    if (b >= count) return;
    constexpr int NN = N * N;
    double *Pb = P + (long)b * NN;
    const int qi = qidx[b];
    const int step = step_of_node ? step_of_node[b] : -1;
    if (qi < 0) {
#pragma unroll
        for (int e = 0; e < NN; ++e) Pb[e] = 0.0;
        if (info) { info[2 * b] = 0; info[2 * b + 1] = 0; }
        if (step >= 0)
#pragma unroll
            for (int e = 0; e < NN; ++e) Pfrag[(long)step * NN + e] = 0.0;
        return;
    }
    const double *Qb = Q + (long)qi * NN;
    const double t = tt[b];
    SmallMat<N> A;
#pragma unroll
    for (int i = 0; i < N; ++i)
#pragma unroll
        for (int j = 0; j < N; ++j) A.a[i][j] = Qb[i * N + j] * t;
    double nrm = 0.0;
#pragma unroll
    for (int j = 0; j < N; ++j) {
        double cs = 0.0;
#pragma unroll
        for (int i = 0; i < N; ++i) cs += fabs(A.a[i][j]);
        nrm = fmax(nrm, cs);
    }
    int m = 13, s = 0;
    if (nrm <= c_theta[0]) m = 3;
    else if (nrm <= c_theta[1]) m = 5;
    else if (nrm <= c_theta[2]) m = 7;
    else if (nrm <= c_theta[3]) m = 9;
    else if (nrm > c_theta[4]) {
        int e;
        const double f = frexp(nrm / c_theta[4], &e);
        s = (f == 0.5) ? e - 1 : e;
        if (s < 0) s = 0;
    }
    if (info) { info[2 * b] = m; info[2 * b + 1] = s; }
    if (s > 0) {
        const double sc = ldexp(1.0, -s);
#pragma unroll
        for (int i = 0; i < N; ++i)
#pragma unroll
            for (int j = 0; j < N; ++j) A.a[i][j] *= sc;
    }
    SmallMat<N> A2, A4, A6, U, V, W, Z;
    sm_comb(Z, 0.0, A, 0.0, A, 0.0, A, 0.0);
    sm_mul(A, A, A2);
    A4 = Z; A6 = Z;
    if (m >= 5) sm_mul(A2, A2, A4);
    if (m >= 7) sm_mul(A4, A2, A6);
    if (m == 13) {
        sm_comb(W, c_b13[13], A6, c_b13[11], A4, c_b13[9], A2, 0.0);
        sm_mul(A6, W, W);
        sm_comb(U, c_b13[7], A6, c_b13[5], A4, c_b13[3], A2, c_b13[1]);
        sm_comb(W, 1.0, W, 1.0, U, 0.0, Z, 0.0);
        sm_mul(A, W, U);
        sm_comb(W, c_b13[12], A6, c_b13[10], A4, c_b13[8], A2, 0.0);
        sm_mul(A6, W, W);
// ... 48 lines not shown
#pragma unroll
        for (int j = 0; j < N; ++j) {
            double acc = X.a[k][j];
#pragma unroll
            for (int i = k + 1; i < N; ++i) acc = fma(-M.a[k][i], X.a[i][j], acc);
            X.a[k][j] = acc * rinv;
        }
    }
    for (int q = 0; q < s; ++q) sm_mul(X, X, X);
    if (singular) {
        if (info) info[2 * b] = -1;
#pragma unroll
        for (int i = 0; i < N; ++i)
#pragma unroll
            for (int j = 0; j < N; ++j) X.a[i][j] = __builtin_nan("");
    }
#pragma unroll
    for (int i = 0; i < N; ++i)
#pragma unroll
        for (int j = 0; j < N; ++j) {
            Pb[i * N + j] = X.a[i][j];
            if (step >= 0) Pfrag[(long)step * NN + i * N + j] = X.a[i][j];
        }
}

template <int N>
__global__ void __launch_bounds__(256)
expm_small_taylor_kernel(int count, const double *__restrict__ Q, const int *__restrict__ qidx,
                         const double *__restrict__ tt, double *__restrict__ P,
                         int *__restrict__ info, const int *__restrict__ step_of_node,
                         double *__restrict__ Pfrag, rt_reduce_args red)
{
    if (red.partial && blockIdx.x == gridDim.x - 1) {
        rt_reduce_partials_body(red.partial, red.npartials, red.totals, red.nsites);
        return;
    }
    const int b = blockIdx.x * 256 + threadIdx.x;
    if (b >= count) return;
    constexpr int NN = N * N;
    double *Pb = P + (long)b * NN;
    const int qi = qidx[b];
    const int step = step_of_node ? step_of_node[b] : -1;
    const double t = tt[b];
    SmallMat<N> A;
#pragma unroll
    for (int i = 0; i < N; ++i)
#pragma unroll
        for (int j = 0; j < N; ++j) A.a[i][j] = Q[i * N + j];
    if (qi < 0) {
#pragma unroll
        for (int e = 0; e < NN; ++e) Pb[e] = 0.0;
        if (info) { info[2 * b] = 0; info[2 * b + 1] = 0; }
        if (step >= 0)
#pragma unroll
            for (int e = 0; e < NN; ++e) Pfrag[(long)step * NN + e] = 0.0;
        return;
    }
    if (qi > 0) {
        const double *Qb = Q + (long)qi * NN;
#pragma unroll
        for (int i = 0; i < N; ++i)
#pragma unroll
            for (int j = 0; j < N; ++j) A.a[i][j] = Qb[i * N + j];
    }
#pragma unroll
    for (int i = 0; i < N; ++i)
#pragma unroll
        for (int j = 0; j < N; ++j) A.a[i][j] *= t;
    SmallMat<N> X;
    int m, s;
    rt_expm_small_taylor<N>(A, X, m, s);
    if (info) { info[2 * b] = m; info[2 * b + 1] = s; }
#pragma unroll
    for (int i = 0; i < N; ++i)
#pragma unroll
        for (int j = 0; j < N; ++j) {
            Pb[i * N + j] = X.a[i][j];
            if (step >= 0) Pfrag[(long)step * NN + i * N + j] = X.a[i][j];
        }
}

}

int64_t rt_expm_carry_groups(rt_ctx *ctx, int64_t n, int64_t count, bool with_reduce, bool quad)
{
    if (n <= 48 || n > 64 || count <= 0) return 0;
    const char *which = getenv("RAOTEH_EXPM");
    if (n <= 62 && which && strcmp(which, "pade") == 0) return 0;
    const char *wv8 = getenv("RAOTEH_EXPM_WAVES");
    if (wv8 && atoi(wv8) == 4) return 0;
    bool split2 = 2 * count + (with_reduce ? 1 : 0) <= (int64_t)std::max(2, ctx->num_cus) && !quad;
    if (const char *v = getenv("RAOTEH_EXPM_SPLIT")) split2 = !quad && atoi(v) != 0;
    return split2 ? 2 * count : count;
}

int rt_launch_expm(rt_ctx *ctx, int64_t n, int64_t count, const double *d_Q,
                   const int32_t *d_qidx, const double *d_t, double *d_P,
                   int32_t *d_info, const int32_t *d_step_of_node, int frag_kind,
                   double *d_Pfrag, const rt_reduce_args *fused_reduce, double *d_Pquad,
                   int64_t variant_count, const rt_combine_args *carried_combine)
{
    const rt_combine_args comb = carried_combine ? *carried_combine : rt_combine_args();
    const int64_t vcount = variant_count > 0 ? variant_count : count;
    const rt_reduce_args red = fused_reduce ? *fused_reduce : rt_reduce_args();
    const unsigned extra = red.partial ? 1u : 0u;
    if (n < 1 || n > RT_MAX_EXPM_STATES) {
        rt_set_error("expm: n=%lld outside 1..%d", (long long)n, RT_MAX_EXPM_STATES);
        return RT_ERR_UNSUPPORTED;
    }
    const int64_t RT_MAX_PADE_STATES = 62;
    RT_REQUIRE(!comb.halfbuf || (variant_count <= 0 &&
                                 comb.nblocks16 <= 4 * rt_expm_carry_groups(ctx, n, count, extra != 0,
                                                                            d_Pquad != nullptr)),
               "expm: this launch cannot carry a root combine");
    if (count <= 0 && !extra) return RT_OK;
    const int ld = (int)n | 1;
    const size_t lds = (size_t)5 * n * ld * 8 + (128 + 128 + 64) * 8 + (8 + 64) * 4;
    size_t &attr_lds = ctx->expm_attr_lds;
    if (n <= RT_MAX_PADE_STATES && lds > attr_lds) {
        RT_HIP(hipFuncSetAttribute((const void *)expm_kernel,
                                   hipFuncAttributeMaxDynamicSharedMemorySize,
                                   (int)lds));
        attr_lds = lds;
    }
    if (n <= 4 && !getenv("RAOTEH_EXPM_NO_SMALL")) {
        hipEvent_t ev = nullptr;
        const char *wh = getenv("RAOTEH_EXPM");
        const bool pade = wh && strcmp(wh, "pade") == 0;
        rt_time_begin(ctx, RT_K_EXPM, pade ? "expm_small_lane_per_matrix_pade"
                                           : "expm_small_lane_per_matrix", &ev);
        const unsigned grid = (unsigned)((count + 255) / 256) + extra;
        const int *son = frag_kind == 0 ? d_step_of_node : nullptr;
        if (!pade) {
#define RT_SMALLT(NV)                                                                \
            RT_LAUNCH_TIMED(ctx, expm_small_taylor_kernel<NV>, dim3(grid), dim3(256), 0, \
                            (int)count, d_Q, d_qidx, d_t, d_P, d_info, son, d_Pfrag, red)
            switch ((int)n) {
            case 1: RT_SMALLT(1); break;
            case 2: RT_SMALLT(2); break;
            case 3: RT_SMALLT(3); break;
            default: RT_SMALLT(4); break;
            }
#undef RT_SMALLT
            RT_HIP(hipGetLastError());
            rt_time_end(ctx, RT_K_EXPM, ev);
            return RT_OK;
        }
#define RT_SMALL(NV)                                                                 \
        RT_LAUNCH_TIMED(ctx, expm_small_kernel<NV>, dim3(grid), dim3(256), 0, \
                           (int)count, d_Q, d_qidx, d_t, d_P, d_info, son, d_Pfrag, red)
        switch ((int)n) {
        case 1: RT_SMALL(1); break;
        case 2: RT_SMALL(2); break;
        case 3: RT_SMALL(3); break;
        default: RT_SMALL(4); break;
        }
#undef RT_SMALL
        RT_HIP(hipGetLastError());
        rt_time_end(ctx, RT_K_EXPM, ev);
        return RT_OK;
    }
    const char *which = getenv("RAOTEH_EXPM");
    if (n > RT_MAX_PADE_STATES || !(which && strcmp(which, "pade") == 0)) {
        const int nt = (int)((n + 15) / 16);
        const size_t msz = (size_t)(16 * nt) * (16 * nt + 1);
        const bool global = nt > 4;
        const size_t lds_t = global ? 0 : 4 * msz * 8;
        double *scratch = nullptr;
        if (global) {
            const size_t need = (size_t)count * 4 * msz * 8;
            if (need > ctx->expm_scratch_bytes) {
                RT_HIP(hipStreamSynchronize(ctx->stream));
                hipFree(ctx->d_expm_scratch);
                ctx->d_expm_scratch = nullptr;
                ctx->expm_scratch_bytes = 0;
                RT_HIP(hipMalloc((void **)&ctx->d_expm_scratch, need));
                ctx->expm_scratch_bytes = need;
            }
            scratch = ctx->d_expm_scratch;
        }
        const char *wv = getenv("RAOTEH_EXPM_WIDE");
        if (global && !(wv && atoi(wv) == 0) && !d_Pquad) {
            bool split2 = 2 * vcount + extra <= (int64_t)std::max(2, ctx->num_cus);
            if (const char *v = getenv("RAOTEH_EXPM_SPLIT")) split2 = atoi(v) != 0;
            const size_t wgs = (size_t)count * (split2 ? 2 : 1);
            const size_t need = wgs * ((nt + 1) / 2) * 4 * nt * 256 * 8;
            if (need > ctx->expm_scratch_bytes) {
                RT_HIP(hipStreamSynchronize(ctx->stream));
                hipFree(ctx->d_expm_scratch);
                ctx->d_expm_scratch = nullptr;
                ctx->expm_scratch_bytes = 0;
                RT_HIP(hipMalloc((void **)&ctx->d_expm_scratch, need));
                ctx->expm_scratch_bytes = need;
            }
            RT_TRY(rt_expm_wide_launch(ctx, nt, split2, wgs + extra, n, d_Q, d_qidx, d_t, d_P, d_info,
                                       d_step_of_node, frag_kind, d_Pfrag, red));
            return RT_OK;
        }
        hipEvent_t ev = nullptr;
        rt_time_begin(ctx, RT_K_EXPM, global ? "expm_taylor_ps_mfma_global" : "expm_taylor_ps_mfma",
                      &ev);
#define RT_TAYLOR(NTV, GL)                                                                      \
        do {                                                                                    \
            if (lds_t > ctx->expm_ts_attr_lds[NTV - 1]) {                                       \
                RT_HIP(hipFuncSetAttribute((const void *)expm_taylor_kernel<NTV, GL>,           \
                                           hipFuncAttributeMaxDynamicSharedMemorySize,          \
                                           (int)lds_t));                                        \
                ctx->expm_ts_attr_lds[NTV - 1] = lds_t;                                         \
            }                                                                                   \
            RT_LAUNCH_TIMED(ctx, (expm_taylor_kernel<NTV, GL>), dim3((unsigned)count + extra),  \
                            dim3(TPB), lds_t, (int)n, d_Q, d_qidx, d_t, d_P, d_info,            \
                            d_step_of_node, frag_kind, d_Pfrag, d_Pquad, scratch, red);         \
        } while (0)
#define RT_TAYLOR8(NTV, SP, SLOT)                                                               \
        do {                                                                                    \
            if (lds_t > ctx->expm_w8_attr_lds[SLOT]) {                                          \
                RT_HIP(hipFuncSetAttribute((const void *)expm_taylor_kernel<NTV, false, SP, 8>, \
                                           hipFuncAttributeMaxDynamicSharedMemorySize,          \
                                           (int)lds_t));                                        \
                ctx->expm_w8_attr_lds[SLOT] = lds_t;                                            \
            }                                                                                   \
            RT_LAUNCH_TIMED(ctx, (expm_taylor_kernel<NTV, false, SP, 8>),                       \
                            dim3((SP ? 2u : 1u) * (unsigned)count + extra), dim3(512), lds_t,   \
                            (int)n, d_Q, d_qidx, d_t, d_P, d_info, d_step_of_node, frag_kind,   \
                            d_Pfrag, d_Pquad, scratch, red);                                    \
        } while (0)
#define RT_TAYLOR8C(SP, SLOT)                                                                   \
        do {                                                                                    \
            if (lds_t > ctx->expm_w8_attr_lds[SLOT]) {                                          \
                RT_HIP(hipFuncSetAttribute((const void *)expm_taylor_carry_kernel<4, false, SP, 8>,          \
                                           hipFuncAttributeMaxDynamicSharedMemorySize,          \
                                           (int)lds_t));                                        \
                ctx->expm_w8_attr_lds[SLOT] = lds_t;                                            \
            }                                                                                   \
            RT_LAUNCH_TIMED(ctx, (expm_taylor_carry_kernel<4, false, SP, 8>),                                \
                            dim3((SP ? 2u : 1u) * (unsigned)count + extra), dim3(512), lds_t,   \
                            (int)n, d_Q, d_qidx, d_t, d_P, d_info, d_step_of_node, frag_kind,   \
                            d_Pfrag, d_Pquad, scratch, red, comb);                              \
        } while (0)
        const char *wv8 = getenv("RAOTEH_EXPM_WAVES");
        const bool waves8 = (nt == 3 || nt == 4) && !(wv8 && atoi(wv8) == 4);
        bool split2 = nt == 4 && 2 * vcount + extra <= (int64_t)std::max(2, ctx->num_cus) && !d_Pquad;
        if (const char *v = getenv("RAOTEH_EXPM_SPLIT")) split2 = nt == 4 && !d_Pquad && atoi(v) != 0;
        if (split2 && waves8) {
            snprintf(ctx->slots[RT_K_EXPM].name, sizeof(ctx->slots[RT_K_EXPM].name),
                     "expm_taylor_ps_mfma_split2");
            RT_TAYLOR8C(true, 2);
        } else if (split2) {
            if (lds_t > ctx->expm_split_attr_lds) {
                RT_HIP(hipFuncSetAttribute((const void *)expm_taylor_kernel<4, false, true>,
                                           hipFuncAttributeMaxDynamicSharedMemorySize, (int)lds_t));
                ctx->expm_split_attr_lds = lds_t;
            }
            snprintf(ctx->slots[RT_K_EXPM].name, sizeof(ctx->slots[RT_K_EXPM].name),
                     "expm_taylor_ps_mfma_split2");
            RT_LAUNCH_TIMED(ctx, (expm_taylor_kernel<4, false, true>),
                            dim3(2u * (unsigned)count + extra), dim3(TPB), lds_t, (int)n, d_Q, d_qidx,
                            d_t, d_P, d_info, d_step_of_node, frag_kind, d_Pfrag, d_Pquad, scratch,
                            red);
        } else
        switch (nt) {
        case 1: RT_TAYLOR(1, false); break;
        case 2: RT_TAYLOR(2, false); break;
        case 3: if (waves8) RT_TAYLOR8(3, false, 0); else RT_TAYLOR(3, false); break;
        case 4: if (waves8) RT_TAYLOR8C(false, 1); else RT_TAYLOR(4, false); break;
        case 5: RT_TAYLOR(5, true); break;
        case 6: RT_TAYLOR(6, true); break;
        case 7: RT_TAYLOR(7, true); break;
        default: RT_TAYLOR(8, true); break;
        }
#undef RT_TAYLOR
#undef RT_TAYLOR8
#undef RT_TAYLOR8C
        RT_HIP(hipGetLastError());
        if (getenv("RAOTEH_EXPM_TRACE")) {
            static int armed = 0;
            unsigned long long tr[8];
            RT_HIP(hipStreamSynchronize(ctx->stream));
            if (armed) {
                RT_HIP(hipMemcpyFromSymbol(tr, HIP_SYMBOL(rt_expm_trace), sizeof tr));
                unsigned long long fn[8];
                RT_HIP(hipMemcpyFromSymbol(fn, HIP_SYMBOL(rt_expm_fine), sizeof fn));
                fprintf(stderr, "[raoteh_amd] last Horner half product: seed + first operands %llu, k loop "
                        "%llu, barrier %llu, write-back %llu, barrier %llu\n", fn[1] - fn[0],
                        fn[2] - fn[1], fn[3] - fn[2], fn[4] - fn[3], fn[5] - fn[4]);
                fprintf(stderr, "[raoteh_amd] expm trace (clocks, workgroup 1): load + norm %llu, order %llu, "
                        "A^2 A^3 %llu, block %llu, Horner %llu, squarings %llu, store %llu; total %llu\n",
                        tr[1] - tr[0], tr[2] - tr[1], tr[3] - tr[2], tr[4] - tr[3], tr[5] - tr[4],
                        tr[6] - tr[5], tr[7] - tr[6], tr[7] - tr[0]);
            }
            const int on = 1;
            RT_HIP(hipMemcpyToSymbol(HIP_SYMBOL(rt_expm_trace_on), &on, sizeof on));
            armed = 1;
        }
        rt_time_end(ctx, RT_K_EXPM, ev);
        return RT_OK;
    }
    hipEvent_t ev = nullptr;
    rt_time_begin(ctx, RT_K_EXPM, "expm_mfma_regsolve", &ev);
    RT_LAUNCH_TIMED(ctx, expm_kernel, dim3((unsigned)count + extra), dim3(TPB), lds,
                       (int)n, d_Q, d_qidx, d_t, d_P, d_info, d_step_of_node, frag_kind,
                       d_Pfrag, d_Pquad, red);
    RT_HIP(hipGetLastError());
    rt_time_end(ctx, RT_K_EXPM, ev);
    return RT_OK;
}
```

### raoteh_amd/csrc/expm_taylor_body.inc

```
{
    extern __shared__ __attribute__((aligned(16))) unsigned char smem[];
    if (red.partial && blockIdx.x == gridDim.x - 1) {
        rt_reduce_partials_body(red.partial, red.npartials, red.totals, red.nsites);
        return;
    }
#if RT_EXPM_CARRY
    static_assert(WAVES == 8 && NT == 4, "the carrying forms: eight waves, 49 <= n <= 64");
    if (comb.halfbuf) {
        const int cw = __builtin_amdgcn_readfirstlane((int)(threadIdx.x >> 6)) - 4;
        if (cw >= 0) {
            const long G = (long)gridDim.x - (red.partial ? 1 : 0);
            const long tile = rt_carry_tile((long)blockIdx.x, cw, G, comb.nblocks16);
            if (tile >= 0) rt_combine_tile_body<4>(comb, tile);
        }
    }
#endif
    constexpr int RN = 16 * NT;
    constexpr int LD = RN + 1;
    constexpr int MSZ = RN * LD;
    __shared__ double colsum[RN];
    const int trace_on = rt_expm_trace_on;
    RT_EXPM_STAMP(0);
    double *B0 = GLOBAL ? scratch + (size_t)blockIdx.x * 4 * MSZ : (double *)smem;
    double *B1 = B0 + MSZ;
    double *B2 = B1 + MSZ;
    double *B3 = B2 + MSZ;

    static_assert(!SPLIT || (NT == 4 && !GLOBAL), "two workgroups per matrix: 49 <= n <= 64");
    static_assert(WAVES == 4 || (WAVES == 8 && !GLOBAL && (NT == 3 || NT == 4)),
                  "two waves per SIMD: LDS-resident, 33 <= n <= 64");
    constexpr int NTH = 64 * WAVES;
    const int b = SPLIT ? (int)(blockIdx.x >> 1) : (int)blockIdx.x;
    const int half = SPLIT ? (int)(blockIdx.x & 1) : 0;
    const int tid = threadIdx.x;
    const int nn = n * n;
    const int KSn = (n + 3) / 4, NTn = (n + 15) / 16;
    double *Pb = P + (long)b * nn;
    const int qi = qidx[b];
    const int step = step_of_node ? step_of_node[b] : -1;
    constexpr int RP0 = GLOBAL ? 1 : TPB / RN;
    constexpr int PER0 = GLOBAL ? 1 : (RN + RP0 - 1) / RP0;
    double q0[PER0];
    if (!GLOBAL) {
        const int jc = tid % RN, g = tid / RN;
#pragma unroll
        for (int u = 0; u < PER0; ++u) {
            const int i = g + u * RP0;
            q0[u] = (g < RP0 && i < n && jc < n) ? Q[i * n + jc] : 0.0;
        }
    }
    const double t_early = tt[b];
    if (qi < 0) {
        for (int e = tid; e < nn; e += NTH) Pb[e] = 0.0;
        if (info && tid == 0) { info[2 * b] = 0; info[2 * b + 1] = 0; }
        if (step >= 0 && frag_kind == 0)
            for (int e = tid; e < nn; e += NTH) Pfrag[(long)step * nn + e] = 0.0;
        if (step >= 0 && frag_kind == 1) {
            const int total = NTn * ((KSn + 1) / 2) * 128;
            for (int e = tid; e < total; e += NTH) Pfrag[(long)step * total + e] = 0.0;
            if (Pquad)
                for (int e = tid; e < KSn * KSn * 16; e += NTH)
                    Pquad[(long)step * rt_quad_stride(n) + e] = 0.0;
        }
        return;
    }
    const double *Qb = Q + (long)qi * nn;
    const double t = t_early;
    double nrm = 0.0;
    if (!GLOBAL) {
        constexpr int RP = TPB / RN;
        constexpr int PER = (RN + RP - 1) / RP;
        __shared__ double colpart[RP][RN];
        const int jc = tid % RN, g = tid / RN;
        const bool active = g < RP;
        double v[PER];
        double part = 0.0;
        if (qi > 0) {
#pragma unroll
            for (int u = 0; u < PER; ++u) {
                const int i = g + u * RP;
                q0[u] = (active && i < n && jc < n) ? Qb[i * n + jc] : 0.0;
            }
        }
#pragma unroll
        for (int u = 0; u < PER; ++u) v[u] = q0[u] * t;
#pragma unroll
        for (int u = 0; u < PER; ++u) {
            const int i = g + u * RP;
            if (active && i < RN) B0[i * LD + jc] = v[u];
            part += fabs(v[u]);
        }
        if (active) colpart[g][jc] = part;
        __syncthreads();
        if (tid < RN) {
            double sum = 0.0;
#pragma unroll
            for (int r = 0; r < RP; ++r) sum += colpart[r][tid];
            colsum[tid] = sum;
        }
        __syncthreads();
        {
            const int ln = tid & 63;
            nrm = ln < RN ? colsum[ln] : 0.0;
#pragma unroll
            for (int o = 32; o > 0; o >>= 1) nrm = fmax(nrm, __shfl_xor(nrm, o, 64));
        }
    } else {
        constexpr int PER = (MSZ + TPB - 1) / TPB;
        for (int c0 = 0; c0 < PER; c0 += 8) {
            double v[8];
#pragma unroll
            for (int u = 0; u < 8; ++u) {
                const int e = (c0 + u) * TPB + tid;
                const int i = e / LD, jx = e - i * LD;
                v[u] = (e < MSZ && i < n && jx < n) ? Qb[i * n + jx] * t : 0.0;
            }
#pragma unroll
            for (int u = 0; u < 8; ++u) {
                const int e = (c0 + u) * TPB + tid;
                if (e < MSZ) B0[e] = v[u];
            }
        }
        __syncthreads();
        for (int jx = tid; jx < RN; jx += TPB) {
            double sum = 0.0;
            for (int i = 0; i < n; ++i) sum += fabs(B0[i * LD + jx]);
            colsum[jx] = sum;
        }
        __syncthreads();
        for (int jj = 0; jj < RN; ++jj) nrm = fmax(nrm, colsum[jj]);
    }
    RT_EXPM_STAMP(1);
    if (!(nrm < 1e300)) {
        for (int e = tid; e < nn; e += NTH) Pb[e] = __builtin_nan("");
        if (info && tid == 0) { info[2 * b] = -1; info[2 * b + 1] = 0; }
        return;
    }
    int m = 15, s = 0;
    if (nrm <= c_theta_taylor[0]) m = 3;
    else if (nrm <= c_theta_taylor[1]) m = 6;
    else if (nrm <= c_theta_taylor[2]) m = 9;
    else if (nrm <= c_theta_taylor[3]) m = 12;
    else if (nrm > c_theta_taylor[4]) {
        int e;
        const double f = frexp(nrm / c_theta_taylor[4], &e);
        s = (f == 0.5) ? e - 1 : e;
        if (s < 0) s = 0;
    }
    m = __builtin_amdgcn_readfirstlane(m);
    s = __builtin_amdgcn_readfirstlane(s);
    if (info && tid == 0) { info[2 * b] = m; info[2 * b + 1] = s; }
    if (s > 0) {
        const double sc = ldexp(1.0, -s);
        for (int e = tid; e < MSZ; e += NTH) B0[e] *= sc;
        __syncthreads();
    }
    const int q = m / 3;
    RT_EXPM_STAMP(2);
    if constexpr (WAVES == 8) {
        const int wave = __builtin_amdgcn_readfirstlane(tid >> 6);
        int wm, wj, wn;
        wave8_tiles<NT>(wave, wm, wj, wn);
        constexpr int NCF = NT == 4 ? 2 : 0;
        const double nd = (double)n;
        const double tops8[5] = {c_inv_fact[3 * (q - 1)], c_inv_fact[3 * (q - 1) + 1],
                                 c_inv_fact[3 * (q - 1) + 2], c_inv_fact[m], nd};
        double left[4 * NT];
        half_tiles ra, ra2;
        load_left8<NT>(B0, wm, left);
        load_tiles8<NT>(B0, ra, wm, wj, wn);
        mm8<NT, NCF>(left, B0, B1, wm, wj, wn, false, 0.0, 0.0, 0.0, nd, nullptr, nullptr,
                     &ra2);
        mm8<NT, NCF>(left, B1, B2, wm, wj, wn, false, 0.0, 0.0, 0.0, nd, &ra, &ra2, nullptr,
                     tops8, B3);
        RT_EXPM_STAMP(3);
        RT_EXPM_STAMP(4);
        if (q >= 2) load_left8<NT>(B2, wm, left);
        if (SPLIT && s == 0) {
            if constexpr (SPLIT) {
                const int hj = 2 * half + (wave & 1);
                half_tiles ha, ha2;
                load_tiles8<NT>(B0, ha, wm, hj, 1);
                load_tiles8<NT>(B1, ha2, wm, hj, 1);
#pragma unroll
                for (int u = 3; u >= 0; --u)
                    if (u <= q - 2)
                        mm8<NT, 1>(left, B3, B3, wm, hj, 1, true, c_inv_fact[3 * u],
                                   c_inv_fact[3 * u + 1], c_inv_fact[3 * u + 2], nd, &ha, &ha2,
                                   nullptr, nullptr, nullptr,
                                   trace_on && blockIdx.x == 2 && u == 0);
            }
        } else {
            for (int jj = q - 2; jj >= 0; --jj)
                mm8<NT, NCF>(left, B3, B3, wm, wj, wn, true, c_inv_fact[3 * jj],
                             c_inv_fact[3 * jj + 1], c_inv_fact[3 * jj + 2], nd, &ra, &ra2);
        }
        RT_EXPM_STAMP(5);
        for (int r = 0; r < s; ++r) {
            load_left8<NT>(B3, wm, left);
            mm8<NT, NCF>(left, B3, B3, wm, wj, wn, false, 0.0, 0.0, 0.0, nd, nullptr, nullptr);
        }
    } else {
        lane_tiles<NT> ra, ra2;
        load_tiles<NT>(B0, ra);
        mm_blocked<NT>(B0, B0, B1, nullptr, nullptr, nullptr, nullptr, nullptr, &ra2);
        __shared__ double tops[5];
        {
            const int base = 3 * (q - 1);
            if (tid == 0) {
                tops[0] = c_inv_fact[base];
                tops[1] = c_inv_fact[base + 1];
                tops[2] = c_inv_fact[base + 2];
                tops[3] = c_inv_fact[m];
                tops[4] = (double)n;
            }
            __syncthreads();
        }
        mm_blocked<NT>(B0, B1, B2, nullptr, nullptr, nullptr, &ra, &ra2, nullptr, tops, B3);
        RT_EXPM_STAMP(3);
        RT_EXPM_STAMP(4);
        __shared__ double cfs_all[5][4];
        if (tid < 20) cfs_all[tid >> 2][tid & 3] = (tid & 3) == 3 ? (double)n
                                                                 : c_inv_fact[3 * (tid >> 2) + (tid & 3)];
        __syncthreads();
        if (SPLIT && s == 0) {
            if constexpr (SPLIT) {
                half_tiles ha, ha2;
                load_half_tiles(B0, ha, half);
                load_half_tiles(B1, ha2, half);
                double hc[4][3];
#pragma unroll
                for (int u = 0; u < 4; ++u)
#pragma unroll
                    for (int e = 0; e < 3; ++e) hc[u][e] = c_inv_fact[3 * u + e];
                const double nd = (double)n;
#pragma unroll
                for (int u = 3; u >= 0; --u)
                    if (u <= q - 2)
                        mm_half(B2, B3, B3, hc[u][0], hc[u][1], hc[u][2], nd, ha, ha2, half,
                                trace_on && blockIdx.x == 2 && u == 0);
            }
        } else {
            for (int jj = q - 2; jj >= 0; --jj)
                mm_blocked<NT>(B2, B3, B3, cfs_all[jj], B0, B1, &ra, &ra2);
        }
        RT_EXPM_STAMP(5);
        for (int r = 0; r < s; ++r) mm_blocked<NT>(B3, B3, B3, nullptr, nullptr, nullptr);
    }
    RT_EXPM_STAMP(6);

    const double *Xb = B3;
    if constexpr (SPLIT) {
        const int jc = 32 * half + (tid & 31), g = tid >> 5;
        if (jc < n)
            for (int i = g; i < n; i += NTH / 32) Pb[i * n + jc] = Xb[i * LD + jc];
        if (step >= 0 && frag_kind == 1) {
            const int KP = (KSn + 1) / 2;
            const int total = NTn * KP * 128;
            for (int blk = tid >> 7; blk < NTn * 4; blk += NTH >> 7) {
                const int mm = blk >> 2, qq = 4 * half + (blk & 3);
                if (qq < KP) {
                    const int e = (mm * KP + qq) * 128 + (tid & 127);
                    const int e2 = e & 1;
                    const int ln = (e >> 1) & 63;
                    const int row = 16 * mm + (ln & 15);
                    const int col = 4 * (2 * qq + e2) + (ln >> 4);
                    Pfrag[(long)step * total + e] = (col < RN) ? Xb[row * LD + col] : 0.0;
                }
            }
        }
        RT_EXPM_STAMP(7);
        return;
    }
    if (!GLOBAL) {
        constexpr int RP = NTH / RN;
        const int jc = tid % RN, g = tid / RN;
        if (g < RP && jc < n)
            for (int i = g; i < n; i += RP) Pb[i * n + jc] = Xb[i * LD + jc];
    } else {
        for (int e = tid; e < nn; e += TPB) {
            const int i = e / n, j = e - i * n;
            Pb[e] = Xb[i * LD + j];
        }
    }
    if (step >= 0 && frag_kind == 0) {
        for (int e = tid; e < nn; e += NTH) {
            const int i = e / n, j = e - i * n;
            Pfrag[(long)step * nn + e] = Xb[i * LD + j];
        }
    } else if (step >= 0 && frag_kind == 1) {
        const int KP = (KSn + 1) / 2;
        const int total = NTn * KP * 128;
        for (int blk = tid >> 7; blk < NTn * KP; blk += NTH >> 7) {
            const int e = blk * 128 + (tid & 127);
            const int e2 = e & 1;
            const int ln = (e >> 1) & 63;
            const int qq = blk % KP;
            const int mm = blk / KP;
            const int row = 16 * mm + (ln & 15);
            const int col = 4 * (2 * qq + e2) + (ln >> 4);
            Pfrag[(long)step * total + e] = (col < RN) ? Xb[row * LD + col] : 0.0;
        }
        if (Pquad) {
            const int tq = KSn * KSn * 16;
            for (int e = tid; e < tq; e += NTH) {
                const int i = e & 3, k = (e >> 2) & 3, blk = e >> 4;
                const int row = 4 * (blk / KSn) + i, col = 4 * (blk % KSn) + k;
                Pquad[(long)step * rt_quad_stride(n) + e] = Xb[row * LD + col];
            }
        }
    }
    RT_EXPM_STAMP(7);
// ... 2 lines not shown
```

### raoteh_amd/csrc/post_common.h

```cpp
#pragma once

#include "common.h"

#include <algorithm>
#include <cmath>
#include <cstdlib>

constexpr double POST_SCRATCH_CAP = 96e9;

struct post_pass {
    const char *who = nullptr;
    rt_model *m = nullptr;
    rt_sites *s = nullptr, *x = nullptr;
    rt_ctx *ctx = nullptr;
    hipStream_t st = nullptr;
    int64_t n = 0, N = 0, nsites = 0;
    bool lane = false, with_D = false;
    bool per_set = false;
    const double *d_cw = nullptr;
    int NT = 0, KS = 0, KP = 0, nops = 0;
    post_plan plan;
    size_t o_L = 0, o_M = 0, o_D = 0, o_status = 0, o_steps = 0, o_ptab = 0, o_PT = 0;
    unsigned char *base = nullptr;
    double *d_L = nullptr, *d_M = nullptr, *d_D = nullptr, *d_PT = nullptr;
// ... 206 lines not shown
    return (m->d_Q || m->spectral) && (int64_t)m->h_t.size() == m->nnodes &&
           (int64_t)m->h_qidx.size() == m->nnodes;
}

struct post_grid {
    int np = 0;
    size_t cnt = 0;
    size_t o_G = 0, o_tau = 0, o_qidx = 0, o_info = 0, o_GT = 0;
    double *d_G = nullptr, *d_GT = nullptr;
    std::vector<double> tau;
    std::vector<int32_t> qidx, info;

    static int check(const post_pass *p, int recompute_transitions, int64_t npoints,
                     const double *lengths, const unsigned char *use_row = nullptr)
    {
        const rt_model *m = p->m;
        RT_REQUIRE(post_model_has_rates(m),
                   "%s: no rates have been set (rt_model_set_rates or "
                   "rt_model_set_rates_spectral; a model with transitions set directly has no rate "
                   "matrix to exponentiate at another length)", p->who);
        RT_REQUIRE(m->rates_current || recompute_transitions,
                   "%s: the transitions were set directly after the rates "
                   "(rt_model_set_transitions): the resident rates and lengths no longer describe them; "
                   "set the rates again or pass recompute_transitions", p->who);
        RT_REQUIRE(lengths, "%s: lengths is NULL", p->who);
        RT_REQUIRE(npoints >= 1 && npoints <= RT_MAX_PROFILE_POINTS,
                   "%s: 1..%d grid points per branch (%lld here)", p->who,
                   RT_MAX_PROFILE_POINTS, (long long)npoints);
        for (int64_t v = 1; v < p->N; ++v)
            for (int64_t g = 0; g < npoints && (!use_row || use_row[v]); ++g) {
                const double x = lengths[v * npoints + g];
                RT_REQUIRE(std::isfinite(x) && x >= 0.0,
                           "%s: length %d of node %lld is negative or not finite", p->who, (int)g,
                           (long long)v);
            }
        return RT_OK;
    }

    int take(post_pass *p, int npoints)
    {
        const rt_model *m = p->m;
        if (m->spectral ? p->n > 64 : p->n > RT_MAX_EXPM_STATES) {
            rt_set_error("%s: n=%lld is beyond what the model's exponential takes", p->who,
                         (long long)p->n);
            return RT_ERR_UNSUPPORTED;
        }
        np = npoints;
        cnt = (size_t)np * p->N;
        const size_t nn = (size_t)p->n * p->n;
        o_G = p->plan.take(cnt * nn * 8);
        o_tau = p->plan.take(cnt * 8);
        o_qidx = p->plan.take(cnt * 4);
        o_info = p->plan.take(cnt * 8);
        o_GT = p->lane ? p->plan.take(8) : p->plan.take((size_t)np * p->nops * p->NT * p->KP * 128 * 8);
        return RT_OK;
    }

    int launch(post_pass *p, const double *lengths, const unsigned char *use_row = nullptr)
    {
        const rt_model *m = p->m;
        const int64_t n = p->n, N = p->N;
        const size_t nn = (size_t)n * n;
        hipStream_t st = p->st;
        d_G = (double *)(p->base + o_G);
        d_GT = (double *)(p->base + o_GT);
        double *d_tau = (double *)(p->base + o_tau);
        int32_t *d_qidx = (int32_t *)(p->base + o_qidx), *d_info = (int32_t *)(p->base + o_info);
        tau.assign(cnt, 0.0);
        qidx.assign(cnt, 0);
        info.assign(2 * cnt, 0);
        for (int k = 0; k < np; ++k)
            for (int64_t v = 0; v < N; ++v) {
                qidx[(size_t)k * N + v] = m->h_qidx[(size_t)v];
                if (v)
                    tau[(size_t)k * N + v] = !use_row || use_row[v] ? lengths[v * np + k] : m->h_t[(size_t)v];
            }
        RT_HIP(hipMemcpyAsync(d_tau, tau.data(), cnt * 8, hipMemcpyHostToDevice, st));
        RT_HIP(hipMemcpyAsync(d_qidx, qidx.data(), cnt * 4, hipMemcpyHostToDevice, st));
        RT_HIP(hipMemsetAsync(d_info, 0, cnt * 8, st));
        if (m->spectral)
            RT_TRY(rt_launch_spectral(p->ctx, n, (int64_t)cnt, m->d_spec, m->d_spec + 2 * nn,
                                      m->d_spec + nn, m->spectral_has_D ? m->d_spec + 2 * nn + n : nullptr,
                                      d_qidx, d_tau, d_G, d_info, nullptr, 0, nullptr));
        else
            RT_TRY(rt_launch_expm(p->ctx, n, (int64_t)cnt, m->d_Q, d_qidx, d_tau, d_G, d_info, nullptr,
                                  0, nullptr));
        RT_HIP(hipMemcpyAsync(info.data(), d_info, cnt * 8, hipMemcpyDeviceToHost, st));
        return RT_OK;
    }

    int pack(post_pass *p)
    {
        const size_t nn = (size_t)p->n * p->n, tab = (size_t)p->nops * p->NT * p->KP * 128;
        for (int k = 0; k < np; ++k)
            RT_TRY(rt_launch_pack_pt(p->ctx, (int)p->n, p->NT, p->KP, p->nops, p->d_ptab,
                                     d_G + (size_t)k * p->N * nn, d_GT + (size_t)k * tab));
        return RT_OK;
    }

    int result(const post_pass *p) const
    {
        for (size_t j = 0; j < cnt; ++j)
            if (info[2 * j] < 0) {
                rt_set_error("%s: expm failed for node %lld at length %g (a non-finite entry or norm "
                             "of tau Q)", p->who, (long long)(j % (size_t)p->N), tau[j]);
                return RT_ERR_SINGULAR;
            }
        return RT_OK;
    }
};


inline int post_fraction_count(const char *who, int64_t nfractions)
{
    RT_REQUIRE(nfractions >= 1 && nfractions <= RT_MAX_PLACE_FRACTIONS,
               "%s: 1..%d fractions (%lld here)", who, RT_MAX_PLACE_FRACTIONS, (long long)nfractions);
    return RT_OK;
}

inline int post_fraction_values(const char *who, int64_t nfractions, const double *fractions)
{
    for (int64_t r = 0; r < nfractions; ++r)
        RT_REQUIRE(std::isfinite(fractions[r]) && fractions[r] >= 0.0 && fractions[r] <= 1.0,
                   "%s: fraction %d is outside [0, 1] or not finite", who, (int)r);
    return RT_OK;
}

inline std::vector<double> post_fraction_lengths(const post_pass *p, int R, const double *fractions,
                                                 int nmore = 0, const double *more = nullptr)
{
    const rt_model *m = p->m;
    const int np = 2 * R + nmore;
    std::vector<double> lengths((size_t)p->N * np, 0.0);
    if (post_model_has_rates(m))
        for (int64_t v = 1; v < p->N; ++v) {
            double *row = lengths.data() + (size_t)v * np;
            const double t = m->h_t[(size_t)v];
            for (int r = 0; r < R; ++r) {
                row[r] = fractions[r] * t;
                row[R + r] = (1.0 - fractions[r]) * t;
            }
            for (int k = 0; k < nmore; ++k) row[2 * R + k] = more[k];
        }
    return lengths;
}

inline int post_fraction_pack(post_pass *p, post_grid *g, int R)
{
    const size_t nn = (size_t)p->n * p->n, tab = (size_t)p->nops * p->NT * p->KP * 128;
    for (int r = 0; r < R; ++r) {
        RT_TRY(rt_launch_pack_pt(p->ctx, (int)p->n, p->NT, p->KP, p->nops, p->d_ptab,
                                 g->d_G + (size_t)r * p->N * nn, g->d_GT + (size_t)r * tab));
        RT_TRY(rt_launch_pack_p(p->ctx, (int)p->n, p->NT, p->KP, p->nops, p->d_ptab,
                                g->d_G + (size_t)(R + r) * p->N * nn, g->d_GT + (size_t)(R + r) * tab));
    }
    return RT_OK;
}


inline int post_class_weights(const char *who, const rt_model *m, const double *class_weights)
{
    const int64_t K = m->multi.K;
    RT_REQUIRE(K >= 1, "%s: the model holds no rate sets (rt_model_set_rate_sets)", who);
    RT_REQUIRE(class_weights, "%s: class_weights is NULL", who);
    bool any = false;
    for (int64_t k = 0; k < K; ++k) {
        const double c = class_weights[k];
        RT_REQUIRE(std::isfinite(c) && c >= 0.0, "class_weights[%lld] is not finite and >= 0",
                   (long long)k);
// ... 30 lines not shown
        return rt_launch_pack_pt(p->ctx, (int)p->n, p->NT, p->KP, (int)(K * p->nops), d_tab, r.d_P, d_PT);
    }
    const double *of_set(int64_t k) const { return d_PT + (size_t)k * (tab / 8); }
};

struct post_set_grid {
    int64_t K = 0;
    int np = 0, nabs = 0;
    size_t o_abs = 0;
    std::vector<double> abs;
    size_t cnt = 0, tab = 0;
    size_t o_G = 0, o_tau = 0, o_qidx = 0, o_info = 0, o_fac = 0, o_GT = 0, o_tab = 0;
    double *d_G = nullptr, *d_GT = nullptr;
    std::vector<double> fac;
    std::vector<int32_t> info, steps;

    static int check(const post_pass *p, int , int64_t npoints,
                     const double *factors, const unsigned char *use_row = nullptr)
    {
        RT_REQUIRE(factors, "%s: factors is NULL", p->who);
        RT_REQUIRE(npoints >= 1 && npoints <= RT_MAX_PROFILE_POINTS,
                   "%s: 1..%d grid points per branch (%lld here)", p->who, RT_MAX_PROFILE_POINTS,
                   (long long)npoints);
        for (int64_t v = 1; v < p->N; ++v)
            for (int64_t g = 0; g < npoints && (!use_row || use_row[v]); ++g) {
                const double x = factors[v * npoints + g];
                RT_REQUIRE(std::isfinite(x) && x >= 0.0,
                           "%s: factor %d of node %lld is negative or not finite", p->who, (int)g,
                           (long long)v);
            }
        return RT_OK;
    }

    int take(post_pass *p, int npoints, int nabsolute = 0)
    {
        if (p->n > RT_MAX_EXPM_STATES) {
            rt_set_error("%s: n=%lld is beyond what the sets' exponential takes", p->who,
                         (long long)p->n);
            return RT_ERR_UNSUPPORTED;
        }
        K = p->m->multi.K; np = npoints; nabs = nabsolute;
        cnt = (size_t)K * np * p->N;
        tab = (size_t)p->nops * p->NT * p->KP * 128;
        const size_t nn = (size_t)p->n * p->n;
        post_plan &plan = p->plan;
        o_G = plan.take(cnt * nn * 8);
        o_tau = plan.take(cnt * 8);
        o_qidx = plan.take(cnt * 4);
        o_info = plan.take(cnt * 8);
        o_fac = plan.take((size_t)p->N * np * 8);
        o_GT = p->lane ? plan.take(8) : plan.take((size_t)K * np * tab * 8);
        o_tab = plan.take((size_t)K * np * p->nops * 4);
        if (nabs) o_abs = plan.take((size_t)(nabs + K) * 8);
        return RT_OK;
    }

    int launch(post_pass *p, const double *factors, const unsigned char *use_row = nullptr,
               const double *abs_tau = nullptr, const double *abs_scale = nullptr)
    {
        RT_REQUIRE(p->d_cw, "%s: the class weights are not on the device yet (post_mix::begin)", p->who);
        const rt_rate_sets &r = p->m->multi;
        const int64_t N = p->N;
        hipStream_t st = p->st;
        d_G = (double *)(p->base + o_G);
        d_GT = (double *)(p->base + o_GT);
        double *d_tau = (double *)(p->base + o_tau), *d_fac = (double *)(p->base + o_fac);
        int32_t *d_qidx = (int32_t *)(p->base + o_qidx), *d_info = (int32_t *)(p->base + o_info);
        fac.assign((size_t)N * np, 1.0);
        for (int64_t v = 1; v < N; ++v)
            for (int g = 0; g < np && (!use_row || use_row[v]); ++g)
                fac[(size_t)(v * np + g)] = factors[v * np + g];
        info.assign(2 * cnt, 0);
        RT_HIP(hipMemcpyAsync(d_fac, fac.data(), fac.size() * 8, hipMemcpyHostToDevice, st));
        RT_HIP(hipMemsetAsync(d_info, 0, cnt * 8, st));
        const double *d_abs = nullptr;
        if (nabs) {
            abs.assign(abs_tau, abs_tau + nabs);
            for (int64_t k = 0; k < K; ++k) abs.push_back(abs_scale ? abs_scale[k] : 1.0);
            d_abs = (const double *)(p->base + o_abs);
            RT_HIP(hipMemcpyAsync(p->base + o_abs, abs.data(), abs.size() * 8, hipMemcpyHostToDevice, st));
        }
        RT_TRY(rt_launch_set_grid_args(p->ctx, (int)K, np, (int)N, r.d_qidx, r.d_t, d_fac, p->d_cw,
                                       nabs, d_abs, d_abs ? d_abs + nabs : nullptr, d_qidx, d_tau));
        RT_TRY(rt_launch_expm(p->ctx, p->n, (int64_t)cnt, r.d_Q, d_qidx, d_tau, d_G, d_info, nullptr, 0,
                              nullptr, nullptr, nullptr, (int64_t)np * N));
        RT_HIP(hipMemcpyAsync(info.data(), d_info, cnt * 8, hipMemcpyDeviceToHost, st));
        return RT_OK;
    }

    int pack(post_pass *p)
    {
        int *d_tab = (int *)(p->base + o_tab);
        const int64_t tables = K * np;
        steps.resize((size_t)tables * p->nops);
        for (int64_t j = 0; j < tables; ++j)
            for (int i = 0; i < p->nops; ++i)
                steps[(size_t)(j * p->nops + i)] = (int32_t)(j * p->N + p->step_node[(size_t)i]);
        RT_HIP(hipMemcpyAsync(d_tab, steps.data(), steps.size() * 4, hipMemcpyHostToDevice, p->st));
        return rt_launch_pack_pt(p->ctx, (int)p->n, p->NT, p->KP, (int)(tables * p->nops), d_tab, d_G, d_GT);
    }

    const double *G_of_set(const post_pass *p, int64_t k) const
    {
        return d_G + (size_t)k * np * p->N * p->n * p->n;
    }
    const double *GT_of_set(int64_t k) const { return d_GT + (size_t)k * np * tab; }

    int result(const post_pass *p) const
    {
        for (size_t j = 0; j < cnt; ++j)
            if (info[2 * j] < 0) {
                rt_set_error("%s: expm failed for node %lld of rate set %lld at point %lld (a "
                             "non-finite entry or norm of tau Q)", p->who,
                             (long long)(j % (size_t)p->N), (long long)(j / ((size_t)np * p->N)),
                             (long long)(j / (size_t)p->N % (size_t)np));
                return RT_ERR_SINGULAR;
            }
        return RT_OK;
    }
};

inline std::vector<double> post_set_fraction_factors(const post_pass *p, int R, const double *fractions,
                                                     int nmore = 0)
{
    const int np = 2 * R + nmore;
    std::vector<double> fac((size_t)p->N * np, 1.0);
    for (int64_t v = 0; v < p->N; ++v)
        for (int r = 0; r < R; ++r) {
            fac[(size_t)(v * np + r)] = v ? fractions[r] : 0.0;
            fac[(size_t)(v * np + R + r)] = v ? 1.0 - fractions[r] : 0.0;
        }
    return fac;
}

struct post_set_fractions {
    int R = 0;
    const post_set_grid *g = nullptr;

    int pack(post_pass *p, post_set_grid *grid, int nfractions)
    {
        g = grid; R = nfractions;
        RT_REQUIRE(g->np >= 2 * R, "%s: the set grid holds %d points, fewer than 2 x %d", p->who, g->np, R);
        int *d_tab = (int *)(p->base + g->o_tab);
        const int64_t K = g->K, half = K * R * p->nops;
        std::vector<int32_t> &steps = grid->steps;
        steps.resize((size_t)(2 * half));
        for (int h = 0; h < 2; ++h)
            for (int64_t k = 0; k < K; ++k)
                for (int r = 0; r < R; ++r)
                    for (int i = 0; i < p->nops; ++i)
                        steps[(size_t)(h * half + (k * R + r) * p->nops + i)] =
                            (int32_t)((k * g->np + h * R + r) * p->N + p->step_node[(size_t)i]);
        RT_HIP(hipMemcpyAsync(d_tab, steps.data(), steps.size() * 4, hipMemcpyHostToDevice, p->st));
        RT_TRY(rt_launch_pack_pt(p->ctx, (int)p->n, p->NT, p->KP, (int)half, d_tab, g->d_G, g->d_GT));
        return rt_launch_pack_p(p->ctx, (int)p->n, p->NT, p->KP, (int)half, d_tab + half, g->d_G,
                                g->d_GT + (size_t)K * R * g->tab);
    }
    const double *T_of_set(int64_t k) const { return g->d_GT + (size_t)k * R * g->tab; }
    const double *A_of_set(int64_t k) const { return g->d_GT + (size_t)(g->K + k) * R * g->tab; }
};

template <int BS>
__global__ void __launch_bounds__(BS)
mix_post_kernel(int K, long nsites, const double *__restrict__ cw, const double *__restrict__ tot,
                const int *__restrict__ set_status, double *__restrict__ post,
                double *__restrict__ loglik, int *__restrict__ status)
{
    const long i = (long)blockIdx.x * BS + threadIdx.x;
// ... 815 lines not shown
```

### raoteh_amd/device.py

```python
from __future__ import annotations

import atexit
import collections
import ctypes
import weakref
from ctypes import byref, c_char_p, c_double, c_int, c_int32, c_int64, c_void_p

import numpy as np

from . import _lib
from ._tree import TreeArrays

__all__ = ['check_rate_sets', 'check_site_sets', 'Context', 'get_context', 'TreeModel', 'SiteBatch', 'device_count', 'Posteriors',
           'states_to_mask', 'BranchExpectations', 'check_branch_coefs', 'SampledStates', 'SampledMappings',
           'MapStates']

_shutting_down = []
atexit.register(_shutting_down.append, True)

_KINDS = {'dense': _lib.RT_OBS_DENSE, 'state': _lib.RT_OBS_STATE,
          'mask': _lib.RT_OBS_MASK}


def _f64(a):
# ... 781 lines not shown
            _lib.lib().rt_sites_destroy(self._h)
            self._h = c_void_p()

    def __del__(self):
        try:
            self.close()
        except Exception:
            pass


class TreeModel(object):

    def __init__(self, T, root, nstates, ctx=None):
        self.ctx = ctx if ctx is not None else get_context()
        self.tree = T if isinstance(T, TreeArrays) else TreeArrays(T, root)
        self.nstates = int(nstates)
        self._h = c_void_p()
        self._batches = weakref.WeakSet()
        self._root_w = None
        ta = self.tree
        _lib.check(_lib.lib().rt_model_create(
            self.ctx._h, ta.nnodes, self.nstates, _ptr(ta.indices, c_int64),
            _ptr(ta.indptr, c_int64), byref(self._h)))
        self.ctx._children.add(self)

    def close(self):
        for batch in list(getattr(self, '_batches', ())):
            batch.close()
        if self._h and not _shutting_down:
            _lib.check(_lib.lib().rt_model_destroy(self._h))
            self._h = c_void_p()

    def __del__(self):
        try:
            self.close()
        except Exception:
            pass

    @property
    def schedule_depth(self):
        return _lib.lib().rt_model_schedule_depth(self._h)

    def set_rates(self, Q_default=None, Q=None, node_q=None, t=None):
        if Q is None:
            Q, node_q = self.tree.rate_matrices(self.nstates, Q_default)
        else:
            Q = _f64(Q)
            if Q.ndim == 2:
                Q = Q[None]
            if Q.shape[1:] != (self.nstates, self.nstates):
                raise ValueError('expected the array to be square')
        if t is None:
            t = self.tree.branch_lengths()
        t = _f64(t)
        nq = _i64(node_q) if node_q is not None else None
        if t.shape != (self.tree.nnodes,):
            raise ValueError('t must have one entry per node')
        _lib.check(_lib.lib().rt_model_set_rates(
            self._h, _ptr(Q, c_double), Q.shape[0],
            None if nq is None else _ptr(nq, c_int64), _ptr(t, c_double)))
        self._rates = (Q.copy(), t.copy())

    def set_rates_spectral(self, A, lam, B, D=None, t=None):
        A, lam, B = _f64(A), _f64(lam), _f64(B)
        n = self.nstates
        if A.shape != (n, n) or B.shape != (n, n) or lam.shape != (n,):
            raise ValueError('expected the array to be square')
        D = None if D is None else _f64(D)
        if D is not None and D.shape != (n,):
            raise ValueError('D must have one entry per state')
        if t is None:
            t = self.tree.branch_lengths()
        t = _f64(t)
        if t.shape != (self.tree.nnodes,):
            raise ValueError('t must have one entry per node')
        _lib.check(_lib.lib().rt_model_set_rates_spectral(
            self._h, _ptr(A, c_double), _ptr(lam, c_double), _ptr(B, c_double),
            None if D is None else _ptr(D, c_double), _ptr(t, c_double)))
        self._rates = None

    def recompute_transitions(self):
        _lib.check(_lib.lib().rt_model_recompute_transitions(self._h))

    def set_transitions(self, esd):
        esd = _f64(esd)
        if esd.shape != (self.tree.nnodes, self.nstates, self.nstates):
            raise ValueError('esd_transitions has the wrong shape')
        _lib.check(_lib.lib().rt_model_set_transitions(self._h,
                                                       _ptr(esd, c_double)))

    def get_transitions(self):
        esd = np.empty((self.tree.nnodes, self.nstates, self.nstates))
        _lib.check(_lib.lib().rt_model_get_transitions(self._h,
                                                       _ptr(esd, c_double)))
        return esd

    def expm_info(self):
        info = np.zeros((self.tree.nnodes, 2), dtype=np.int32)
        _lib.check(_lib.lib().rt_model_get_expm_info(self._h,
                                                     _ptr(info, c_int32)))
        return info

    def set_root_distn(self, root_distn=None):
        if root_distn is None:
            _lib.check(_lib.lib().rt_model_set_root_distn(self._h, None))
            self._root_w = None
            return
        w = _f64(root_distn)
        if w.shape != (self.nstates,):
            raise ValueError('root shape mismatch: %s %s' % (
                (self.nstates,), w.shape))
        _lib.check(_lib.lib().rt_model_set_root_distn(self._h,
                                                      _ptr(w, c_double)))
        self._root_w = w.copy()

    def upload_sites(self, obs_nodes, data, kind='dense', site_sets=None, nsets=None):
        code = _KINDS[kind]
        idx = _i64([self.tree.node_to_index[v] for v in obs_nodes])
        if kind == 'dense':
            data = _f64(data)
            ok = data.ndim == 3 and data.shape[2] == self.nstates
        elif kind == 'state':
            data = _as_uint8_states(data, self.nstates)
            ok = data.ndim == 2
        else:
            data = np.ascontiguousarray(data, dtype=np.uint64)
            words = (self.nstates + 63) // 64
            ok = (data.ndim == 2 and words == 1) or (data.ndim == 3 and data.shape[2] == words)
        if not ok or data.shape[1] != len(idx):
            raise ValueError('observation array has the wrong shape')
        nsites = data.shape[0]
        h = c_void_p()
        if site_sets is not None:
            sets, nsets = check_site_sets(site_sets, nsites, nsets)
            _lib.check(_lib.lib().rt_sites_create_partitioned(
                self._h, nsites, code, len(idx), _ptr(idx, c_int64),
                data.ctypes.data_as(c_void_p), _ptr(sets, c_int32), nsets, byref(h)))
            return SiteBatch(self, h, nsites, sets, nsets)
        _lib.check(_lib.lib().rt_sites_create(
            self._h, nsites, code, len(idx), _ptr(idx, c_int64),
            data.ctypes.data_as(c_void_p), byref(h)))
        batch = SiteBatch(self, h, nsites)
        if self.tree.nnodes == 1:
            batch._host_obs = (kind, idx, data.copy())
        return batch

    def prune(self, batch):
        _lib.check(_lib.lib().rt_prune(self._h, batch._h))

    def step(self, batch, recompute_transitions=True):
        _lib.check(_lib.lib().rt_step(self._h, batch._h,
                                      1 if recompute_transitions else 0))

    def set_rate_sets(self, Q, t=None, node_q=None):
        if t is None:
            t = self.tree.branch_lengths()
        Q, t, node_q = check_rate_sets(Q, t, node_q, self.nstates, self.tree.nnodes)
        _lib.check(_lib.lib().rt_model_set_rate_sets(
            self._h, Q.shape[0], _ptr(Q, c_double), Q.shape[1],
            None if node_q is None else _ptr(node_q, c_int64), _ptr(t, c_double)))
        self._nsets = Q.shape[0]
        self._rate_sets = (Q.copy(), t.copy())

    def step_multi(self, batch, recompute_transitions=True):
        _lib.check(_lib.lib().rt_step_multi(self._h, batch._h,
                                            1 if recompute_transitions else 0))
# ... 687 lines not shown
```

Baseline: 55.92 million sites/s.

## Cache rate-matrix squares and cubes across expm calls for 49-64 state models

```diff
diff --git a/include/raoteh_hip.h b/include/raoteh_hip.h
--- a/include/raoteh_hip.h
+++ b/include/raoteh_hip.h
@@ -159,6 +159,10 @@
 int rt_step(rt_model *model, rt_sites *sites, int recompute_transitions);
 int rt_carry_combine_deal(int64_t nt, int64_t nblocks16, int64_t G, int root_halves,
             int rescale, int partitioned, int multi, int64_t *tile_of);
+int rt_model_qpow_stats(rt_model *m, int64_t *fills, int64_t *hits, int *valid);
+int rt_model_qpow_sets_stats(rt_model *m, int64_t *fills, int64_t *hits, int *valid);
+int rt_expm_qpow_storer_rule(int64_t count, int64_t nq, const int32_t *qidx, const double *t,
+                             const double *qnorm, int32_t *storer);
 int rt_expect_step(rt_model *model, rt_sites *sites, int recompute_transitions,
             double *dwell, double *root_posterior, double *trans, int32_t *status);
 #define RT_MAX_POSTERIOR_SETS 8
diff --git a/raoteh_amd/_lib.py b/raoteh_amd/_lib.py
--- a/raoteh_amd/_lib.py
+++ b/raoteh_amd/_lib.py
@@ -114,6 +114,9 @@
     'rt_model_get_schedule': (c_int, [c_void_p, _p_i32, c_int64, _p_i64]),
     'rt_build_schedule': (c_int, [c_int64, _p_i64, _p_i64, _p_i32, _p_i32]),
     'rt_carry_combine_deal': (c_int, [c_int64, c_int64, c_int64, c_int, c_int, c_int, c_int, _p_i64]),
+    'rt_model_qpow_stats': (c_int, [c_void_p, _p_i64, _p_i64, POINTER(c_int)]),
+    'rt_model_qpow_sets_stats': (c_int, [c_void_p, _p_i64, _p_i64, POINTER(c_int)]),
+    'rt_expm_qpow_storer_rule': (c_int, [c_int64, c_int64, _p_i32, _p_f64, _p_f64, _p_i32]),
     'rt_set_option': (c_int, [c_char_p, c_int64]),
     'rt_ctx_set_option': (c_int, [c_void_p, c_char_p, c_int64]),
     'rt_sites_jit_compile_seconds': (c_double, [c_void_p]),
diff --git a/raoteh_amd/csrc/api.hip b/raoteh_amd/csrc/api.hip
--- a/raoteh_amd/csrc/api.hip
+++ b/raoteh_amd/csrc/api.hip
@@ -377,6 +377,7 @@
 static void rate_sets_release(rt_model *m)
 {
     rt_rate_sets &r = m->multi;
+    rt_qpow_release(r.qpow);
     hipFree(r.d_Q); hipFree(r.d_qidx); hipFree(r.d_t); hipFree(r.d_info); hipFree(r.d_step_of_node);
     hipFree(r.d_P); hipFree(r.d_Pfrag); hipFree(r.d_Pquad); hipFree(r.d_Pcol);
     r = rt_rate_sets();
@@ -396,7 +397,7 @@
     rt_expect_lane_release(m);
     hipStreamSynchronize(m->ctx->stream);
     hipFree(m->d_indices); hipFree(m->d_indptr); hipFree(m->d_ops); hipFree(m->d_P);
-    hipFree(m->d_Pfrag); hipFree(m->d_Pquad); hipFree(m->d_Pcol); hipFree(m->d_root); hipFree(m->d_Q); hipFree(m->d_spec); hipFree(m->d_qidx);
+    hipFree(m->d_Pfrag); hipFree(m->d_Pquad); hipFree(m->d_Pcol); hipFree(m->d_root); hipFree(m->d_Q); rt_qpow_release(m->qpow); hipFree(m->d_spec); hipFree(m->d_qidx);
     hipFree(m->d_t); hipFree(m->d_info); hipFree(m->d_step_of_node);
     hipFree(m->d_qidx_step); hipFree(m->d_t_step);
     rate_sets_release(m);
@@ -503,6 +504,99 @@
     return RT_OK;
 }
 
+int rt_qpow_reserve(rt_qpow_cache &c, int64_t n, int64_t nq)
+{
+    if (n <= 48 || n > 64 || nq <= c.capacity) return RT_OK;
+    rt_qpow_release(c);
+    hipError_t e = hipMalloc((void **)&c.d_pow, (size_t)nq * 2 * n * n * 8);
+    if (e == hipSuccess) e = hipMalloc((void **)&c.d_storer, (size_t)nq * 4);
+    if (e != hipSuccess) {
+        rt_qpow_release(c);
+        rt_set_error("stored powers of the rate matrices: %s", hipGetErrorString(e));
+        return e == hipErrorOutOfMemory ? RT_ERR_NOMEM : RT_ERR_HIP;
+    }
+    c.capacity = nq;
+    return RT_OK;
+}
+
+void rt_qpow_release(rt_qpow_cache &c)
+{
+    hipFree(c.d_pow);
+    hipFree(c.d_storer);
+    c.d_pow = nullptr;
+    c.d_storer = nullptr;
+    c.capacity = 0;
+    c.valid = false;
+}
+
+bool rt_qpow_record(rt_qpow_cache &c, int64_t n, int64_t nq, const double *h_Q, int64_t count,
+                    const int32_t *h_qidx, const double *h_t, rt_expm_powers *pw)
+{
+    if (n <= 48 || n > 64 || !c.d_pow || nq < 1 || nq > c.capacity || !rt_expm_qpow_enabled())
+        return false;
+    pw->d_pow = c.d_pow;
+    pw->d_storer = c.d_storer;
+    pw->mode = c.valid ? RT_QPOW_WARM : RT_QPOW_COLD;
+    if (c.valid) return true;
+    if (!h_Q || !h_qidx || !h_t) return false;
+    std::vector<double> qnorm((size_t)nq);
+    for (int64_t q = 0; q < nq; ++q) {
+        double nrm = 0.0;
+        for (int64_t j = 0; j < n; ++j) {
+            double s = 0.0;
+            for (int64_t i = 0; i < n; ++i) s += std::fabs(h_Q[((size_t)q * n + i) * n + j]);
+            nrm = s > nrm || !(s == s) ? s : nrm;
+        }
+        qnorm[(size_t)q] = nrm;
+    }
+    std::vector<int32_t> storer((size_t)nq);
+    rt_expm_qpow_storers(count, nq, h_qidx, h_t, qnorm.data(), storer.data());
+    bool any = false;
+    for (int32_t v : storer) any = any || v >= 0;
+    if (!any) return false;
+    const hipError_t e = hipMemcpy(c.d_storer, storer.data(), (size_t)nq * 4, hipMemcpyHostToDevice);
+    if (e != hipSuccess) {
+        rt_set_error("stored powers of the rate matrices: copying the storers failed: %s",
+                     hipGetErrorString(e));
+        return false;
+    }
+    return true;
+}
+
+void rt_qpow_launched(rt_qpow_cache &c, const rt_expm_powers &pw, bool have, int rc)
+{
+    if (rc != RT_OK) { c.valid = false; return; }
+    if (!have || !pw.used) return;
+    if (c.valid) ++c.hits;
+    else { c.valid = true; ++c.fills; }
+}
+
+extern "C" int rt_model_qpow_stats(rt_model *m, int64_t *fills, int64_t *hits, int *valid)
+{
+    RT_REQUIRE(m, "null pointer");
+    if (fills) *fills = m->qpow.fills;
+    if (hits) *hits = m->qpow.hits;
+    if (valid) *valid = m->qpow.valid ? 1 : 0;
+    return RT_OK;
+}
+
+extern "C" int rt_model_qpow_sets_stats(rt_model *m, int64_t *fills, int64_t *hits, int *valid)
+{
+    RT_REQUIRE(m, "null pointer");
+    if (fills) *fills = m->multi.qpow.fills;
+    if (hits) *hits = m->multi.qpow.hits;
+    if (valid) *valid = m->multi.qpow.valid ? 1 : 0;
+    return RT_OK;
+}
+
+extern "C" int rt_expm_qpow_storer_rule(int64_t count, int64_t nq, const int32_t *qidx,
+                                        const double *t, const double *qnorm, int32_t *storer)
+{
+    RT_REQUIRE(qidx && storer && count >= 0 && nq >= 0, "bad arguments");
+    rt_expm_qpow_storers(count, nq, qidx, t, qnorm, storer);
+    return RT_OK;
+}
+
 static int model_run_expm(rt_model *m)
 {
     rt_reduce_args red;
@@ -526,9 +620,14 @@
     RT_TRY(rt_take_pending_combine(m->ctx, rt_expm_carry_groups(m->ctx, m->n, m->nnodes, carry,
                                                                 m->d_Pquad != nullptr),
                                    carry ? &red : nullptr, &comb, &carried));
+    rt_expm_powers pw;
+    const bool have_pw = rt_qpow_record(m->qpow, m->n, m->h_nq, m->h_Q.data(), m->nnodes,
+                                        m->h_qidx.data(), m->h_t.data(), &pw);
     const int erc = rt_launch_expm(m->ctx, m->n, m->nnodes, m->d_Q, m->d_qidx, m->d_t, m->d_P,
                                    m->d_info, m->d_step_of_node, m->n <= 4 ? 0 : 1, m->d_Pfrag,
-                                   carry ? &red : nullptr, m->d_Pquad, 0, carried ? &comb : nullptr);
+                                   carry ? &red : nullptr, m->d_Pquad, 0, carried ? &comb : nullptr,
+                                   have_pw ? &pw : nullptr);
+    rt_qpow_launched(m->qpow, pw, have_pw, erc);
     if (carried) RT_TRY(rt_carried_combine_done(m->ctx, carried, erc == RT_OK));
     RT_TRY(erc);
     m->have_P = true;
@@ -567,10 +666,26 @@
         m->q_capacity = 0;
         RT_HIP(hipMalloc((void **)&m->d_Q, nq * nn * 8));
         m->q_capacity = nq;
-    }
+        m->h_Q.clear();
+        m->h_nq = 0;
+        m->qpow.valid = false;
+    }
+    const bool qp = m->n > 48 && m->n <= 64;
+    RT_TRY(rt_qpow_reserve(m->qpow, m->n, m->q_capacity));
     hipStream_t st = m->ctx->stream;
+    const bool same_Q = qp && !m->spectral && nq == m->h_nq && m->h_Q.size() == (size_t)nq * nn &&
+                        memcmp(m->h_Q.data(), Q, (size_t)nq * nn * 8) == 0;
     RT_HIP(hipStreamSynchronize(st));
-    RT_HIP(hipMemcpy(m->d_Q, Q, nq * nn * 8, hipMemcpyHostToDevice));
+    if (!same_Q) {
+        m->qpow.valid = false;
+        m->h_Q.clear();
+        m->h_nq = 0;
+        RT_HIP(hipMemcpy(m->d_Q, Q, nq * nn * 8, hipMemcpyHostToDevice));
+        if (qp) {
+            m->h_Q.assign(Q, Q + (size_t)nq * nn);
+            m->h_nq = nq;
+        }
+    }
     RT_TRY(model_upload_edge_parameters(m, qi, tt));
     m->spectral = false;
     return model_run_expm(m);
@@ -605,6 +720,9 @@
     m->spectral_has_D = D != nullptr;
     RT_TRY(model_upload_edge_parameters(m, qi, tt));
     m->spectral = true;
+    m->qpow.valid = false;
+    m->h_Q.clear();
+    m->h_nq = 0;
     return model_run_expm(m);
 }
 
@@ -731,9 +849,14 @@
 static int rate_sets_run_expm(rt_model *m)
 {
     rt_rate_sets &r = m->multi;
-    RT_TRY(rt_launch_expm(m->ctx, m->n, r.K * m->nnodes, r.d_Q, r.d_qidx, r.d_t, r.d_P, r.d_info,
-                          r.d_step_of_node, m->n <= 4 ? 0 : 1, r.d_Pfrag, nullptr, r.d_Pquad,
-                          m->nnodes));
+    rt_expm_powers pw;
+    const bool have_pw = rt_qpow_record(r.qpow, m->n, r.K * r.nq, r.h_Q.data(), r.K * m->nnodes,
+                                        r.h_qidx.data(), r.h_t.data(), &pw);
+    const int erc = rt_launch_expm(m->ctx, m->n, r.K * m->nnodes, r.d_Q, r.d_qidx, r.d_t, r.d_P,
+                                   r.d_info, r.d_step_of_node, m->n <= 4 ? 0 : 1, r.d_Pfrag, nullptr,
+                                   r.d_Pquad, m->nnodes, nullptr, have_pw ? &pw : nullptr);
+    rt_qpow_launched(r.qpow, pw, have_pw, erc);
+    RT_TRY(erc);
     return rate_sets_pack_pcol(m, true);
 }
 
@@ -775,7 +898,14 @@
     RT_TRY(rate_sets_reserve(m, K, nq));
     rt_rate_sets &r = m->multi;
     RT_HIP(hipStreamSynchronize(m->ctx->stream));
+    r.qpow.valid = false;
+    RT_TRY(rt_qpow_reserve(r.qpow, m->n, r.q_capacity));
     RT_HIP(hipMemcpy(r.d_Q, Q, (size_t)(K * nq) * nn * 8, hipMemcpyHostToDevice));
+    if (m->n > 48 && m->n <= 64) {
+        r.h_Q.assign(Q, Q + (size_t)(K * nq) * nn);
+        r.h_qidx = qi;
+        r.h_t = tt;
+    }
     RT_HIP(hipMemcpy(r.d_qidx, qi.data(), qi.size() * 4, hipMemcpyHostToDevice));
     RT_HIP(hipMemcpy(r.d_t, tt.data(), tt.size() * 8, hipMemcpyHostToDevice));
     if (K != r.K) r.epoch += 1;
diff --git a/raoteh_amd/csrc/common.h b/raoteh_amd/csrc/common.h
--- a/raoteh_amd/csrc/common.h
+++ b/raoteh_amd/csrc/common.h
@@ -136,6 +136,14 @@
     int32_t dst;
 };
 
+struct rt_qpow_cache {
+    double *d_pow = nullptr;
+    int32_t *d_storer = nullptr;
+    int64_t capacity = 0;
+    bool valid = false;
+    int64_t fills = 0, hits = 0;
+};
+
 struct rt_rate_sets {
     int64_t K = 0;
     int64_t capacity = 0;
@@ -151,6 +159,9 @@
     double *d_Pfrag = nullptr, *d_Pquad = nullptr, *d_Pcol = nullptr;
     int64_t pcol_capacity = 0;
     int64_t P_stride = 0, frag_stride = 0, quad_stride = 0, pcol_stride = 0;
+    rt_qpow_cache qpow;
+    std::vector<double> h_Q, h_t;
+    std::vector<int32_t> h_qidx;
 };
 
 struct rt_model {
@@ -174,6 +185,9 @@
     bool spectral = false, spectral_has_D = false;
     double *d_Q = nullptr;
     int64_t q_capacity = 0;
+    rt_qpow_cache qpow;
+    std::vector<double> h_Q;
+    int64_t h_nq = 0;
     int32_t *d_qidx = nullptr;
     double *d_t = nullptr;
     int32_t *d_info = nullptr;
@@ -349,12 +363,42 @@
                         const int *d_qidx, const double *d_t, double *d_P, int *d_info,
                         const int *d_step_of_node, int frag_kind, double *d_Pfrag,
                         const rt_reduce_args &red);
+enum { RT_QPOW_COLD = 0, RT_QPOW_WARM = 1 };
+struct rt_expm_powers {
+    double *d_pow = nullptr;
+    int mode = RT_QPOW_COLD;
+    const int32_t *d_storer = nullptr;
+    bool used = false;
+};
+bool rt_expm_qpow_enabled();
+inline void rt_expm_qpow_storers(int64_t count, int64_t nq, const int32_t *qidx, const double *t,
+                                 const double *qnorm, int32_t *storer)
+{
+    for (int64_t q = 0; q < nq; ++q) storer[q] = -1;
+    for (int64_t b = 0; b < count; ++b) {
+        const int32_t q = qidx[b];
+        if (q < 0 || q >= nq || storer[q] >= 0) continue;
+        if (t && t[b] == 0.0) continue;
+        if (qnorm) {
+            if (!(qnorm[q] >= 1e-85 && qnorm[q] <= 1e85)) continue;
+            const double at = t ? (t[b] < 0 ? -t[b] : t[b]) * qnorm[q] : 1.0;
+            if (!(at >= 1e-250 && at <= 1e250)) continue;
+        }
+        storer[q] = (int32_t)b;
+    }
+}
+int rt_qpow_reserve(rt_qpow_cache &c, int64_t n, int64_t nq);
+bool rt_qpow_record(rt_qpow_cache &c, int64_t n, int64_t nq, const double *h_Q, int64_t count,
+                    const int32_t *h_qidx, const double *h_t, rt_expm_powers *pw);
+void rt_qpow_launched(rt_qpow_cache &c, const rt_expm_powers &pw, bool have, int rc);
+void rt_qpow_release(rt_qpow_cache &c);
 int rt_launch_expm(rt_ctx *ctx, int64_t n, int64_t count, const double *d_Q,
                    const int32_t *d_qidx, const double *d_t, double *d_P,
                    int32_t *d_info, const int32_t *d_step_of_node, int frag_kind,
                    double *d_Pfrag, const rt_reduce_args *fused_reduce = nullptr,
                    double *d_Pquad = nullptr, int64_t variant_count = 0,
-                   const rt_combine_args *carried_combine = nullptr);
+                   const rt_combine_args *carried_combine = nullptr,
+                   rt_expm_powers *powers = nullptr);
 int rt_launch_spectral(rt_ctx *ctx, int64_t n, int64_t count, const double *d_A,
                        const double *d_lam, const double *d_B, const double *d_D,
                        const int32_t *d_qidx, const double *d_t, double *d_P, int32_t *d_info,
diff --git a/raoteh_amd/csrc/expm.hip b/raoteh_amd/csrc/expm.hip
--- a/raoteh_amd/csrc/expm.hip
+++ b/raoteh_amd/csrc/expm.hip
@@ -410,6 +410,35 @@
     1.0 / 40320.0, 1.0 / 362880.0, 1.0 / 3628800.0, 1.0 / 39916800.0, 1.0 / 479001600.0,
     1.0 / 6227020800.0, 1.0 / 87178291200.0, 1.0 / 1307674368000.0};
 
+__device__ __forceinline__ double top_block(const double *top, double r1, double r2, double a3,
+                                            bool diag)
+{
+    double w = top[1] * r1;
+    w = fma(top[2], r2, w);
+    w = fma(top[3], a3, w);
+    return w + (diag ? top[0] : 0.0);
+}
+
+struct qp_tiles {
+    double v[2][4];
+};
+
+__device__ __forceinline__ void qp_load(const double *G, int n, qp_tiles &t)
+{
+    const int lane = threadIdx.x & 63;
+    const int wave = __builtin_amdgcn_readfirstlane(threadIdx.x >> 6);
+    const int lr = lane & 15, lq = lane >> 4;
+#pragma unroll
+    for (int k = 0; k < 2; ++k) {
+        const int col = 16 * (2 * (wave & 1) + k) + lr;
+#pragma unroll
+        for (int r = 0; r < 4; ++r) {
+            const int row = 16 * (wave >> 1) + 4 * r + lq;
+            t.v[k][r] = (row < n && col < n) ? G[row * n + col] : 0.0;
+        }
+    }
+}
+
 template <int NT>
 struct lane_tiles {
     double v[(NT + 1) / 2][(NT + 1) / 2][4];
@@ -436,13 +465,14 @@
         }
 }
 
-template <int NT>
+template <int NT, bool OUT = false>
 __device__ __forceinline__ void mm_blocked(const double *X, const double *Y, double *C,
                                            const double *cf, const double *P1, const double *P2,
                                            const lane_tiles<NT> *R1 = nullptr,
                                            const lane_tiles<NT> *R2 = nullptr,
                                            lane_tiles<NT> *out = nullptr,
-                                           const double *top = nullptr, double *C2 = nullptr)
+                                           const double *top = nullptr, double *C2 = nullptr,
+                                           double *gout = nullptr, int gn = 0)
 {
     constexpr int RH = (NT + 1) / 2;
     constexpr int LD = 16 * NT + 1;
@@ -478,8 +508,8 @@
                     for (int r = 0; r < 4; ++r) {
                         const int row = 16 * m + 4 * r + lq;
                         const int o = row * LD + col;
-                        double w = c1 * (R1 ? R1->v[u][v][r] : P1[o]);
-                        if (R2) w = fma(c2, R2->v[u][v][r], w);
+                        double w = c1 * ((NT == 4 || R1) ? R1->v[u][v][r] : P1[o]);
+                        if (NT == 4 || R2) w = fma(c2, R2->v[u][v][r], w);
                         else if (P2) w = fma(c2, P2[o], w);
                         if (row == col && (double)row < cf[3]) w += c0;
                         acc[u][v][r] = w;
@@ -509,7 +539,7 @@
 #pragma unroll
         for (int u = 0; u < RH; ++u) { a0[u] = a1[u]; b0[u] = b1[u]; a1[u] = a2[u]; b1[u] = b2[u]; }
     }
-    if (out) {
+    if (OUT) {
 #pragma unroll
         for (int u = 0; u < RH; ++u)
 #pragma unroll
@@ -528,12 +558,14 @@
 #pragma unroll
                 for (int r = 0; r < 4; ++r) {
                     const int row = 16 * m + 4 * r + lq;
-                    C[row * LD + col] = acc[u][v][r];
+                    if (NT == 4 && gout && row < gn && col < gn) gout[row * gn + col] = acc[u][v][r];
                     if (top) {
-                        double w = top[1] * R1->v[u][v][r];
-                        w = fma(top[2], R2->v[u][v][r], w);
-                        w = fma(top[3], acc[u][v][r], w);
-                        C2[row * LD + col] = w + ((row == col && (double)row < top[4]) ? top[0] : 0.0);
+                        const double a3 = NT == 4 ? top[5] * acc[u][v][r] : acc[u][v][r];
+                        C[row * LD + col] = a3;
+                        C2[row * LD + col] = top_block(top, R1->v[u][v][r], R2->v[u][v][r], a3,
+                                                       row == col && (double)row < top[4]);
+                    } else {
+                        C[row * LD + col] = acc[u][v][r];
                     }
                 }
             }
@@ -650,7 +682,7 @@
                                     double c2, double nd, const half_tiles *R1,
                                     const half_tiles *R2, half_tiles *out = nullptr,
                                     const double *top = nullptr, double *C2 = nullptr,
-                                    bool fine = false)
+                                    bool fine = false, double *gout = nullptr, int gn = 0)
 {
     RT_FINE(0);
     constexpr int LD = 16 * NT + 1, KS = 4 * NT;
@@ -706,16 +738,29 @@
 #pragma unroll
             for (int r = 0; r < 4; ++r) {
                 const int row = 16 * m + 4 * r + lq;
-                C[row * LD + col] = acc[v][r];
                 if (top) {
-                    double w = top[1] * R1->v[v][r];
-                    w = fma(top[2], R2->v[v][r], w);
-                    w = fma(top[3], acc[v][r], w);
-                    C2[row * LD + col] = w + ((row == col && (double)row < top[4]) ? top[0] : 0.0);
+                    const double a3 = NT == 4 ? top[5] * acc[v][r] : acc[v][r];
+                    C[row * LD + col] = a3;
+                    C2[row * LD + col] = top_block(top, R1->v[v][r], R2->v[v][r], a3,
+                                                   row == col && (double)row < top[4]);
+                } else {
+                    C[row * LD + col] = acc[v][r];
                 }
             }
         }
     RT_FINE(4);
+    if (NT == 4 && gout) {
+#pragma unroll
+        for (int v = 0; v < 2; ++v)
+            if (v < nc) {
+                const int col = 16 * (j0 + v) + lr;
+#pragma unroll
+                for (int r = 0; r < 4; ++r) {
+                    const int row = 16 * m + 4 * r + lq;
+                    if (row < gn && col < gn) gout[row * gn + col] = acc[v][r];
+                }
+            }
+    }
     __syncthreads();
     RT_FINE(5);
 }
@@ -732,7 +777,7 @@
                    const double *__restrict__ tt, double *__restrict__ P,
                    int *__restrict__ info, const int *__restrict__ step_of_node,
                    int frag_kind, double *__restrict__ Pfrag, double *__restrict__ Pquad,
-                   double *__restrict__ scratch, rt_reduce_args red)
+                   double *__restrict__ scratch, rt_reduce_args red, rt_expm_powers pw)
 #define RT_EXPM_CARRY 0
 #include "expm_taylor_body.inc"
 #undef RT_EXPM_CARRY
@@ -743,7 +788,8 @@
                          const double *__restrict__ tt, double *__restrict__ P,
                          int *__restrict__ info, const int *__restrict__ step_of_node,
                          int frag_kind, double *__restrict__ Pfrag, double *__restrict__ Pquad,
-                         double *__restrict__ scratch, rt_reduce_args red, rt_combine_args comb)
+                         double *__restrict__ scratch, rt_reduce_args red, rt_combine_args comb,
+                         rt_expm_powers pw)
 #define RT_EXPM_CARRY 1
 #include "expm_taylor_body.inc"
 #undef RT_EXPM_CARRY
@@ -958,6 +1004,12 @@
 
 }
 
+bool rt_expm_qpow_enabled()
+{
+    const char *v = getenv("RAOTEH_EXPM_QPOW");
+    return !(v && atoi(v) == 0);
+}
+
 int64_t rt_expm_carry_groups(rt_ctx *ctx, int64_t n, int64_t count, bool with_reduce, bool quad)
 {
     if (n <= 48 || n > 64 || count <= 0) return 0;
@@ -974,8 +1026,10 @@
                    const int32_t *d_qidx, const double *d_t, double *d_P,
                    int32_t *d_info, const int32_t *d_step_of_node, int frag_kind,
                    double *d_Pfrag, const rt_reduce_args *fused_reduce, double *d_Pquad,
-                   int64_t variant_count, const rt_combine_args *carried_combine)
-{
+                   int64_t variant_count, const rt_combine_args *carried_combine,
+                   rt_expm_powers *powers)
+{
+    if (powers) powers->used = false;
     const rt_combine_args comb = carried_combine ? *carried_combine : rt_combine_args();
     const int64_t vcount = variant_count > 0 ? variant_count : count;
     const rt_reduce_args red = fused_reduce ? *fused_reduce : rt_reduce_args();
@@ -1041,6 +1095,11 @@
         const int nt = (int)((n + 15) / 16);
         const size_t msz = (size_t)(16 * nt) * (16 * nt + 1);
         const bool global = nt > 4;
+        rt_expm_powers pw;
+        if (powers && nt == 4 && powers->d_pow && powers->d_storer && rt_expm_qpow_enabled()) {
+            pw = *powers;
+            powers->used = true;
+        }
         const size_t lds_t = global ? 0 : 4 * msz * 8;
         double *scratch = nullptr;
         if (global) {
@@ -1086,7 +1145,7 @@
             }                                                                                   \
             RT_LAUNCH_TIMED(ctx, (expm_taylor_kernel<NTV, GL>), dim3((unsigned)count + extra),  \
                             dim3(TPB), lds_t, (int)n, d_Q, d_qidx, d_t, d_P, d_info,            \
-                            d_step_of_node, frag_kind, d_Pfrag, d_Pquad, scratch, red);         \
+                            d_step_of_node, frag_kind, d_Pfrag, d_Pquad, scratch, red, pw);     \
         } while (0)
 #define RT_TAYLOR8(NTV, SP, SLOT)                                                               \
         do {                                                                                    \
@@ -1099,7 +1158,7 @@
             RT_LAUNCH_TIMED(ctx, (expm_taylor_kernel<NTV, false, SP, 8>),                       \
                             dim3((SP ? 2u : 1u) * (unsigned)count + extra), dim3(512), lds_t,   \
                             (int)n, d_Q, d_qidx, d_t, d_P, d_info, d_step_of_node, frag_kind,   \
-                            d_Pfrag, d_Pquad, scratch, red);                                    \
+                            d_Pfrag, d_Pquad, scratch, red, pw);                                \
         } while (0)
 #define RT_TAYLOR8C(SP, SLOT)                                                                   \
         do {                                                                                    \
@@ -1112,7 +1171,7 @@
             RT_LAUNCH_TIMED(ctx, (expm_taylor_carry_kernel<4, false, SP, 8>),                                \
                             dim3((SP ? 2u : 1u) * (unsigned)count + extra), dim3(512), lds_t,   \
                             (int)n, d_Q, d_qidx, d_t, d_P, d_info, d_step_of_node, frag_kind,   \
-                            d_Pfrag, d_Pquad, scratch, red, comb);                              \
+                            d_Pfrag, d_Pquad, scratch, red, comb, pw);                          \
         } while (0)
         const char *wv8 = getenv("RAOTEH_EXPM_WAVES");
         const bool waves8 = (nt == 3 || nt == 4) && !(wv8 && atoi(wv8) == 4);
@@ -1133,7 +1192,7 @@
             RT_LAUNCH_TIMED(ctx, (expm_taylor_kernel<4, false, true>),
                             dim3(2u * (unsigned)count + extra), dim3(TPB), lds_t, (int)n, d_Q, d_qidx,
                             d_t, d_P, d_info, d_step_of_node, frag_kind, d_Pfrag, d_Pquad, scratch,
-                            red);
+                            red, pw);
         } else
         switch (nt) {
         case 1: RT_TAYLOR(1, false); break;
diff --git a/raoteh_amd/csrc/expm_taylor_body.inc b/raoteh_amd/csrc/expm_taylor_body.inc
--- a/raoteh_amd/csrc/expm_taylor_body.inc
+++ b/raoteh_amd/csrc/expm_taylor_body.inc
@@ -15,6 +15,15 @@
         }
     }
 #endif
+    constexpr bool QP = NT == 4 && !GLOBAL;
+    qp_tiles pq2 = {}, pq3 = {};
+    const bool pw_warm = QP && pw.mode == RT_QPOW_WARM && pw.d_pow != nullptr;
+    if constexpr (QP && WAVES == 8) {
+        if (pw_warm) {
+            qp_load(pw.d_pow, n, pq2);
+            qp_load(pw.d_pow + n * n, n, pq3);
+        }
+    }
     constexpr int RN = 16 * NT;
     constexpr int LD = RN + 1;
     constexpr int MSZ = RN * LD;
@@ -66,6 +75,14 @@
     }
     const double *Qb = Q + (long)qi * nn;
     const double t = t_early;
+    int pw_edge = -1;
+    if constexpr (QP) {
+        if (pw.d_storer) pw_edge = pw.d_storer[qi];
+        if (WAVES == 8 && pw_warm && qi > 0) {
+            qp_load(pw.d_pow + (long)qi * 2 * nn, n, pq2);
+            qp_load(pw.d_pow + ((long)qi * 2 + 1) * nn, n, pq3);
+        }
+    }
     double nrm = 0.0;
     if (!GLOBAL) {
         constexpr int RP = TPB / RN;
@@ -87,7 +104,7 @@
 #pragma unroll
         for (int u = 0; u < PER; ++u) {
             const int i = g + u * RP;
-            if (active && i < RN) B0[i * LD + jc] = v[u];
+            if (active && i < RN) B0[i * LD + jc] = QP ? q0[u] : v[u];
             part += fabs(v[u]);
         }
         if (active) colpart[g][jc] = part;
@@ -150,11 +167,33 @@
     m = __builtin_amdgcn_readfirstlane(m);
     s = __builtin_amdgcn_readfirstlane(s);
     if (info && tid == 0) { info[2 * b] = m; info[2 * b + 1] = s; }
-    if (s > 0) {
+    double qt = 1.0, qs = 1.0, tau2 = 1.0, tau3 = 1.0;
+    bool warm = false, store = false;
+    if constexpr (QP) {
+        const double at = fabs(t);
+        const int guard = __builtin_amdgcn_readfirstlane(
+            (int)(t == 0.0 || !(nrm >= 1e-90 * at && nrm <= 1e90 * at)));
+        const double sc = ldexp(1.0, -s);
+        if (guard) {
+            for (int e = tid; e < MSZ; e += NTH) B0[e] = (B0[e] * t) * sc;
+            __syncthreads();
+        } else {
+            const double tau = t * sc;
+            qt = t;
+            qs = sc;
+            tau2 = tau * tau;
+            tau3 = tau2 * tau;
+            warm = __builtin_amdgcn_readfirstlane((int)(pw_warm && pw_edge >= 0)) != 0;
+            store = __builtin_amdgcn_readfirstlane(
+                        (int)(!pw_warm && pw.d_pow && pw_edge == b && half == 0)) != 0;
+        }
+    } else if (s > 0) {
         const double sc = ldexp(1.0, -s);
         for (int e = tid; e < MSZ; e += NTH) B0[e] *= sc;
         __syncthreads();
     }
+    double *const g2 = store ? pw.d_pow + (long)qi * 2 * nn : nullptr;
+    double *const g3 = store ? g2 + nn : nullptr;
     const int q = m / 3;
     RT_EXPM_STAMP(2);
     if constexpr (WAVES == 8) {
@@ -163,16 +202,50 @@
         wave8_tiles<NT>(wave, wm, wj, wn);
         constexpr int NCF = NT == 4 ? 2 : 0;
         const double nd = (double)n;
-        const double tops8[5] = {c_inv_fact[3 * (q - 1)], c_inv_fact[3 * (q - 1) + 1],
-                                 c_inv_fact[3 * (q - 1) + 2], c_inv_fact[m], nd};
+        const double tops8[6] = {c_inv_fact[3 * (q - 1)], c_inv_fact[3 * (q - 1) + 1],
+                                 c_inv_fact[3 * (q - 1) + 2], c_inv_fact[m], nd, tau3};
         double left[4 * NT];
         half_tiles ra, ra2;
-        load_left8<NT>(B0, wm, left);
+        const bool products = !(QP && warm);
+        if (products) load_left8<NT>(B0, wm, left);
         load_tiles8<NT>(B0, ra, wm, wj, wn);
-        mm8<NT, NCF>(left, B0, B1, wm, wj, wn, false, 0.0, 0.0, 0.0, nd, nullptr, nullptr,
-                     &ra2);
-        mm8<NT, NCF>(left, B1, B2, wm, wj, wn, false, 0.0, 0.0, 0.0, nd, &ra, &ra2, nullptr,
-                     tops8, B3);
+        if constexpr (QP) {
+#pragma unroll
+            for (int v = 0; v < 2; ++v)
+#pragma unroll
+                for (int r = 0; r < 4; ++r) ra.v[v][r] = (ra.v[v][r] * qt) * qs;
+        }
+        if (!products) {
+            if constexpr (QP && WAVES == 8) {
+                const int lr = tid & 15, lq = (tid & 63) >> 4;
+#pragma unroll
+                for (int v = 0; v < 2; ++v) {
+                    const int col = 16 * (wj + v) + lr;
+#pragma unroll
+                    for (int r = 0; r < 4; ++r) {
+                        const int row = 16 * wm + 4 * r + lq;
+                        ra2.v[v][r] = tau2 * pq2.v[v][r];
+                        const double a3 = tops8[5] * pq3.v[v][r];
+                        B1[row * LD + col] = pq2.v[v][r];
+                        B2[row * LD + col] = a3;
+                        B3[row * LD + col] = top_block(tops8, ra.v[v][r], ra2.v[v][r], a3,
+                                                       row == col && (double)row < tops8[4]);
+                    }
+                }
+                __syncthreads();
+            }
+        } else {
+            mm8<NT, NCF>(left, B0, B1, wm, wj, wn, false, 0.0, 0.0, 0.0, nd, nullptr, nullptr,
+                         &ra2, nullptr, nullptr, false, g2, n);
+            if constexpr (QP) {
+#pragma unroll
+                for (int v = 0; v < 2; ++v)
+#pragma unroll
+                    for (int r = 0; r < 4; ++r) ra2.v[v][r] = tau2 * ra2.v[v][r];
+            }
+            mm8<NT, NCF>(left, B1, B2, wm, wj, wn, false, 0.0, 0.0, 0.0, nd, &ra, &ra2, nullptr,
+                         tops8, B3, false, g3, n);
+        }
         RT_EXPM_STAMP(3);
         RT_EXPM_STAMP(4);
         if (q >= 2) load_left8<NT>(B2, wm, left);
@@ -183,6 +256,11 @@
                 load_tiles8<NT>(B0, ha, wm, hj, 1);
                 load_tiles8<NT>(B1, ha2, wm, hj, 1);
 #pragma unroll
+                for (int r = 0; r < 4; ++r) {
+                    ha.v[0][r] = (ha.v[0][r] * qt) * qs;
+                    ha2.v[0][r] = tau2 * ha2.v[0][r];
+                }
+#pragma unroll
                 for (int u = 3; u >= 0; --u)
                     if (u <= q - 2)
                         mm8<NT, 1>(left, B3, B3, wm, hj, 1, true, c_inv_fact[3 * u],
@@ -203,8 +281,16 @@
     } else {
         lane_tiles<NT> ra, ra2;
         load_tiles<NT>(B0, ra);
-        mm_blocked<NT>(B0, B0, B1, nullptr, nullptr, nullptr, nullptr, nullptr, &ra2);
-        __shared__ double tops[5];
+        constexpr int RHQ = (NT + 1) / 2;
+        if constexpr (QP) {
+#pragma unroll
+            for (int u = 0; u < RHQ; ++u)
+#pragma unroll
+                for (int v = 0; v < RHQ; ++v)
+#pragma unroll
+                    for (int r = 0; r < 4; ++r) ra.v[u][v][r] = (ra.v[u][v][r] * qt) * qs;
+        }
+        __shared__ double tops[6];
         {
             const int base = 3 * (q - 1);
             if (tid == 0) {
@@ -213,10 +299,51 @@
                 tops[2] = c_inv_fact[base + 2];
                 tops[3] = c_inv_fact[m];
                 tops[4] = (double)n;
+                tops[5] = tau3;
             }
             __syncthreads();
         }
-        mm_blocked<NT>(B0, B1, B2, nullptr, nullptr, nullptr, &ra, &ra2, nullptr, tops, B3);
+        if (QP && warm) {
+            if constexpr (QP && WAVES == 4) {
+                const double *G2 = pw.d_pow + (long)qi * 2 * nn, *G3 = G2 + nn;
+                const int lr = tid & 15, lq = (tid & 63) >> 4;
+                const int wr = __builtin_amdgcn_readfirstlane(tid >> 7);
+                const int wc = __builtin_amdgcn_readfirstlane((tid >> 6) & 1);
+#pragma unroll
+                for (int u = 0; u < 2; ++u)
+#pragma unroll
+                    for (int v = 0; v < 2; ++v) {
+                        const int col = 16 * (2 * wc + v) + lr;
+#pragma unroll
+                        for (int r = 0; r < 4; ++r) {
+                            const int row = 16 * (2 * wr + u) + 4 * r + lq;
+                            const bool in = row < n && col < n;
+                            const double q2 = in ? G2[row * n + col] : 0.0;
+                            const double q3 = in ? G3[row * n + col] : 0.0;
+                            ra2.v[u][v][r] = tau2 * q2;
+                            const double a3 = tops[5] * q3;
+                            B1[row * LD + col] = q2;
+                            B2[row * LD + col] = a3;
+                            B3[row * LD + col] = top_block(tops, ra.v[u][v][r], ra2.v[u][v][r], a3,
+                                                           row == col && (double)row < tops[4]);
+                        }
+                    }
+                __syncthreads();
+            }
+        } else {
+            mm_blocked<NT, true>(B0, B0, B1, nullptr, nullptr, nullptr, nullptr, nullptr, &ra2, nullptr,
+                           nullptr, g2, n);
+            if constexpr (QP) {
+#pragma unroll
+                for (int u = 0; u < RHQ; ++u)
+#pragma unroll
+                    for (int v = 0; v < RHQ; ++v)
+#pragma unroll
+                        for (int r = 0; r < 4; ++r) ra2.v[u][v][r] = tau2 * ra2.v[u][v][r];
+            }
+            mm_blocked<NT>(B0, B1, B2, nullptr, nullptr, nullptr, &ra, &ra2, nullptr, tops, B3,
+                           g3, n);
+        }
         RT_EXPM_STAMP(3);
         RT_EXPM_STAMP(4);
         __shared__ double cfs_all[5][4];
@@ -228,6 +355,13 @@
                 half_tiles ha, ha2;
                 load_half_tiles(B0, ha, half);
                 load_half_tiles(B1, ha2, half);
+#pragma unroll
+                for (int v = 0; v < 2; ++v)
+#pragma unroll
+                    for (int r = 0; r < 4; ++r) {
+                        ha.v[v][r] = (ha.v[v][r] * qt) * qs;
+                        ha2.v[v][r] = tau2 * ha2.v[v][r];
+                    }
                 double hc[4][3];
 #pragma unroll
                 for (int u = 0; u < 4; ++u)
diff --git a/raoteh_amd/csrc/post_common.h b/raoteh_amd/csrc/post_common.h
--- a/raoteh_amd/csrc/post_common.h
+++ b/raoteh_amd/csrc/post_common.h
@@ -312,9 +312,17 @@
             RT_TRY(rt_launch_spectral(p->ctx, n, (int64_t)cnt, m->d_spec, m->d_spec + 2 * nn,
                                       m->d_spec + nn, m->spectral_has_D ? m->d_spec + 2 * nn + n : nullptr,
                                       d_qidx, d_tau, d_G, d_info, nullptr, 0, nullptr));
-        else
-            RT_TRY(rt_launch_expm(p->ctx, n, (int64_t)cnt, m->d_Q, d_qidx, d_tau, d_G, d_info, nullptr,
-                                  0, nullptr));
+        else {
+            rt_qpow_cache &qc = const_cast<rt_model *>(m)->qpow;
+            rt_expm_powers pw;
+            const bool have_pw = rt_qpow_record(qc, n, m->h_nq, m->h_Q.data(), (int64_t)cnt,
+                                                qidx.data(), tau.data(), &pw);
+            const int erc = rt_launch_expm(p->ctx, n, (int64_t)cnt, m->d_Q, d_qidx, d_tau, d_G, d_info,
+                                           nullptr, 0, nullptr, nullptr, nullptr, 0, nullptr,
+                                           have_pw ? &pw : nullptr);
+            rt_qpow_launched(qc, pw, have_pw, erc);
+            RT_TRY(erc);
+        }
         RT_HIP(hipMemcpyAsync(info.data(), d_info, cnt * 8, hipMemcpyDeviceToHost, st));
         return RT_OK;
     }
@@ -511,8 +519,15 @@
         }
         RT_TRY(rt_launch_set_grid_args(p->ctx, (int)K, np, (int)N, r.d_qidx, r.d_t, d_fac, p->d_cw,
                                        nabs, d_abs, d_abs ? d_abs + nabs : nullptr, d_qidx, d_tau));
-        RT_TRY(rt_launch_expm(p->ctx, p->n, (int64_t)cnt, r.d_Q, d_qidx, d_tau, d_G, d_info, nullptr, 0,
-                              nullptr, nullptr, nullptr, (int64_t)np * N));
+        rt_qpow_cache &qc = const_cast<rt_model *>(p->m)->multi.qpow;
+        rt_expm_powers pw;
+        const bool have_pw = qc.valid && rt_qpow_record(qc, p->n, r.K * r.nq, nullptr, 0, nullptr,
+                                                        nullptr, &pw);
+        const int erc = rt_launch_expm(p->ctx, p->n, (int64_t)cnt, r.d_Q, d_qidx, d_tau, d_G, d_info,
+                                       nullptr, 0, nullptr, nullptr, nullptr, (int64_t)np * N, nullptr,
+                                       have_pw ? &pw : nullptr);
+        rt_qpow_launched(qc, pw, have_pw, erc);
+        RT_TRY(erc);
         RT_HIP(hipMemcpyAsync(info.data(), d_info, cnt * 8, hipMemcpyDeviceToHost, st));
         return RT_OK;
     }
diff --git a/raoteh_amd/device.py b/raoteh_amd/device.py
--- a/raoteh_amd/device.py
+++ b/raoteh_amd/device.py
@@ -887,6 +887,12 @@
     def recompute_transitions(self):
         _lib.check(_lib.lib().rt_model_recompute_transitions(self._h))
 
+    def qpow_stats(self, sets=False):
+        fills, hits, valid = c_int64(0), c_int64(0), ctypes.c_int(0)
+        fn = _lib.lib().rt_model_qpow_sets_stats if sets else _lib.lib().rt_model_qpow_stats
+        _lib.check(fn(self._h, ctypes.byref(fills), ctypes.byref(hits), ctypes.byref(valid)))
+        return {'fills': fills.value, 'hits': hits.value, 'valid': bool(valid.value)}
+
     def set_transitions(self, esd):
         esd = _f64(esd)
         if esd.shape != (self.tree.nnodes, self.nstates, self.nstates):
```

New measurement: 56.82 million sites/s, median of 6. +1.6%, better.
